# NTHU-LSALAB/KubeShare

Measured on AMD Instinct MI355X. Metric: aggregate images/sec, co-located shared-GPU pods, higher is better.
Workload: dtype bf16; 1 GPU; model=resnet50, global_batch=512, image_size=224, parallelism=2 pods @ request=0.5, 2/GPU, pods_per_gpu=2, miopen_find=False, lease_accounting=sampled-busy

## Files before the change

kubeshare_amd/models/resnet.py:

```python
from __future__ import annotations

import torch
import torch.nn as nn

from .conv import LowpConv2d
from .pool import FusedMaxPool2d


class Bottleneck(nn.Module):
    expansion = 4
    fused_ops = False

    def __init__(self, in_ch: int, width: int, stride: int = 1):
        super().__init__()
        out_ch = width * self.expansion
        self.conv1 = LowpConv2d(in_ch, width, 1, bias=False)
        self.bn1 = nn.BatchNorm2d(width)
        self.conv2 = LowpConv2d(width, width, 3, stride=stride, padding=1,
                                bias=False)
        self.bn2 = nn.BatchNorm2d(width)
        self.conv3 = LowpConv2d(width, out_ch, 1, bias=False)
        self.bn3 = nn.BatchNorm2d(out_ch)
        self.relu = nn.ReLU(inplace=True)
        self.down = None
        if stride != 1 or in_ch != out_ch:
            self.down = nn.Sequential(
                LowpConv2d(in_ch, out_ch, 1, stride=stride, bias=False),
                nn.BatchNorm2d(out_ch),
            )

    def forward(self, x):
        pair = isinstance(x, tuple)
        x, x_id = x if pair else (x, x)
        if self.fused_ops:
            from .. import ops
            identity = x_id if self.down is None else \
                ops.bn_relu(self.down[0](x_id), self.down[1], relu=False)
            out = ops.bn_relu(self.conv1(x), self.bn1)
            out = ops.bn_relu(self.conv2(out), self.bn2)
            return ops.bn_relu(self.conv3(out), self.bn3, res=identity,
                               fork=pair)
        identity = x_id if self.down is None else self.down(x_id)
        out = self.relu(self.bn1(self.conv1(x)))
        out = self.relu(self.bn2(self.conv2(out)))
        out = self.bn3(self.conv3(out))
        out = self.relu(out + identity)
        return (out, out) if pair else out


class BasicBlock(nn.Module):
    expansion = 1
    fused_ops = False

    def __init__(self, in_ch: int, width: int, stride: int = 1):
        super().__init__()
        self.conv1 = LowpConv2d(in_ch, width, 3, stride=stride, padding=1,
                                bias=False)
        self.bn1 = nn.BatchNorm2d(width)
        self.conv2 = LowpConv2d(width, width, 3, padding=1, bias=False)
        self.bn2 = nn.BatchNorm2d(width)
        self.relu = nn.ReLU(inplace=True)
        self.down = None
        if stride != 1 or in_ch != width:
            self.down = nn.Sequential(
                LowpConv2d(in_ch, width, 1, stride=stride, bias=False),
                nn.BatchNorm2d(width),
            )

    def forward(self, x):
        pair = isinstance(x, tuple)
        x, x_id = x if pair else (x, x)
        if self.fused_ops:
            from .. import ops
            identity = x_id if self.down is None else \
                ops.bn_relu(self.down[0](x_id), self.down[1], relu=False)
            out = ops.bn_relu(self.conv1(x), self.bn1)
            return ops.bn_relu(self.conv2(out), self.bn2, res=identity,
                               fork=pair)
        identity = x_id if self.down is None else self.down(x_id)
        out = self.relu(self.bn1(self.conv1(x)))
        out = self.bn2(self.conv2(out))
        out = self.relu(out + identity)
        return (out, out) if pair else out


class ResNet(nn.Module):
    fused_ops = False

    def __init__(self, block, layers, num_classes: int = 1000):
        super().__init__()
        self.in_ch = 64
        self.conv1 = LowpConv2d(3, 64, 7, stride=2, padding=3, bias=False)
        self.bn1 = nn.BatchNorm2d(64)
        self.relu = nn.ReLU(inplace=True)
        self.maxpool = FusedMaxPool2d(3, stride=2, padding=1)
        self.layer1 = self._make_layer(block, 64, layers[0])
        self.layer2 = self._make_layer(block, 128, layers[1], stride=2)
        self.layer3 = self._make_layer(block, 256, layers[2], stride=2)
        self.layer4 = self._make_layer(block, 512, layers[3], stride=2)
        self.avgpool = nn.AdaptiveAvgPool2d(1)
        self.fc = nn.Linear(512 * block.expansion, num_classes)
        for m in self.modules():
            if isinstance(m, nn.Conv2d):
                nn.init.kaiming_normal_(m.weight, mode="fan_out",
                                        nonlinearity="relu")
            elif isinstance(m, nn.BatchNorm2d):
                nn.init.ones_(m.weight)
                nn.init.zeros_(m.bias)
        self._lowp_convs = [m for m in self.modules()
                            if isinstance(m, LowpConv2d)]

    def _make_layer(self, block, width, n, stride=1):
        layers = [block(self.in_ch, width, stride)]
        self.in_ch = width * block.expansion
        layers += [block(self.in_ch, width) for _ in range(n - 1)]
        return nn.Sequential(*layers)

    def forward(self, x):
        if not self.fused_ops:
            return self._forward(x)
        from .. import ops
        staged = ops.stage_lowp_weights(self._lowp_convs)
        try:
            return self._forward(x)
        finally:
            ops.clear_lowp_weights(staged)

    def _forward(self, x):
        if self.fused_ops:
            from .. import ops
            x = self.maxpool(ops.PendingBNReLU(self.conv1(x), self.bn1))
            if ops.bn_fork_enabled():
                x = (x, x)
        else:
            x = self.maxpool(self.relu(self.bn1(self.conv1(x))))
        x = self.layer4(self.layer3(self.layer2(self.layer1(x))))
        if isinstance(x, tuple):
            x = x[0]
        x = torch.flatten(self.avgpool(x), 1)
        return self.fc(x)


def resnet18(num_classes: int = 1000) -> ResNet:
    return ResNet(BasicBlock, [2, 2, 2, 2], num_classes)


def resnet50(num_classes: int = 1000) -> ResNet:
    return ResNet(Bottleneck, [3, 4, 6, 3], num_classes)
```

kubeshare_amd/ops/__init__.py:

```python
from __future__ import annotations

import os

_HERE = os.path.dirname(os.path.abspath(__file__))
_BUILD_DIR = os.path.join(_HERE, "_build")
_SRCS = [os.path.join(_HERE, "hip", "ks_ops.hip"),
         os.path.join(_HERE, "hip", "bn_relu.hip"),
         os.path.join(_HERE, "hip", "pool.hip"),
         os.path.join(_HERE, "hip", "bn_pool.hip"),
         os.path.join(_HERE, "hip", "bias_relu.hip"),
         os.path.join(_HERE, "hip", "cast.hip")]

_ext = None


def build_extension(verbose: bool = False):
    import torch
    from torch.utils import cpp_extension

    os.environ.setdefault("PYTORCH_ROCM_ARCH", "gfx950")
    os.makedirs(_BUILD_DIR, exist_ok=True)
    return cpp_extension.load(
        name="ks_ops",
        sources=_SRCS,
        build_directory=_BUILD_DIR,
        extra_cflags=["-O3"],
        verbose=verbose,
        is_python_module=True,
    )


def _load():
    global _ext
    if _ext is not None:
        return _ext
    import torch

    so = os.path.join(_BUILD_DIR, "ks_ops.so")
    if os.path.exists(so):
        import importlib.util

        spec = importlib.util.spec_from_file_location("ks_ops", so)
        mod = importlib.util.module_from_spec(spec)
        spec.loader.exec_module(mod)
        _ext = mod
        return _ext
    if torch.cuda.is_available():
        _ext = build_extension()
        return _ext
    raise ImportError(
        "kubeshare_amd.ops extension not built; run __graft_entry__.build()")


def burn(ms: float, blocks: int = 1024, threads: int = 256):
    _load().burn(float(ms), blocks, threads)


class FusedSGD:

    def __init__(self, params, lr: float, momentum: float = 0.9,
                 weight_decay: float = 0.0, graph_mode: str = "auto"):
        import torch

        self.params = [p for p in params if p.requires_grad]
        self.lr = lr
        self.momentum = momentum
        self.weight_decay = weight_decay
        self.momenta = [torch.zeros_like(p) for p in self.params]
        self._graph_mode = graph_mode
        self._multi = os.environ.get("KUBESHARE_SGD_MULTI", "1") != "0"
        self._step_graph = None
        self._graph_ptrs = None

    def _graphable(self):
        import torch
        if self._graph_mode == "off" or not torch.cuda.is_available():
            return False
        if os.environ.get("KUBESHARE_SGD_GRAPH", "1") == "0":
            return False
        return all(p.grad is not None and p.grad.is_cuda
                   for p in self.params)

    def _ptrs(self):
        return tuple(
            (p.data_ptr(), v.data_ptr(),
             p.grad.data_ptr() if p.grad is not None else 0)
            for p, v in zip(self.params, self.momenta))

    def zero_grad(self, set_to_none: bool = True):
        for p in self.params:
            if set_to_none:
                p.grad = None
            elif p.grad is not None:
                p.grad.zero_()

    def _launch(self):
        ext = _load()
        if self._multi:
            ext.sgd_momentum_multi_(
                [p.data for p in self.params],
                [p.grad for p in self.params], self.momenta,
                self.lr, self.momentum, self.weight_decay)
            return
        ps, gs, vs = [], [], []
        for p, v in zip(self.params, self.momenta):
            if p.grad is None:
                continue
            ps.append(p.data)
            gs.append(p.grad)
            vs.append(v)
        ext.sgd_momentum_(ps, gs, vs, self.lr, self.momentum,
                          self.weight_decay)

    def _capture(self):
        import torch
        ptrs = self._ptrs()
        step_g = torch.cuda.CUDAGraph()
        with torch.cuda.graph(step_g):
            self._launch()
        self._step_graph = step_g
        self._graph_ptrs = ptrs

    def step(self):
        if self._step_graph is not None and \
                self._graph_ptrs == self._ptrs():
            self._step_graph.replay()
            return
        self._launch()
        if self._step_graph is None and self._graph_mode == "auto" and \
                self._graphable():
            try:
                self._capture()
            except Exception:
                self._graph_mode = "off"


def _bn_relu_autograd():
    global _BNReLUFn
    if _BNReLUFn is not None:
        return _BNReLUFn
    import torch

    class BNReLUFn(torch.autograd.Function):

        @staticmethod
        def forward(ctx, x, res, weight, bias, running_mean, running_var,
                    training, momentum, eps, relu, fork=False):
            ext = _load()
            w32 = weight.float()
            b32 = bias.float()
            ctx.set_materialize_grads(False)
            ctx.with_res = res is not None
            ctx.relu = relu
            ctx.wdtype = weight.dtype
            ctx.legacy_reduce = bn_reduce_legacy()
            if training:
                y, mean, invstd = ext.bn_relu_fwd_train(
                    x, w32, b32, running_mean, running_var, momentum, eps,
                    res, relu, ctx.legacy_reduce)
                ctx.save_for_backward(x, y, w32, b32, mean, invstd)
            else:
                y = ext.bn_relu_fwd_eval(x, w32, b32, running_mean.float(),
                                         running_var.float(), eps, res, relu)
                ctx.save_for_backward(x, y, w32, b32, running_mean.float(),
                                      (running_var.float() + eps).rsqrt())
            return (y, y.view_as(y)) if fork else y

        @staticmethod
        def backward(ctx, dy, dy2=None):
            ext = _load()
            x, y, w32, b32, mean, invstd = ctx.saved_tensors
            if dy is None:
                dy, dy2 = dy2, None
            if dy is None:
                return (None,) * 11
            out = ext.bn_relu_bwd(x, y, dy, w32, b32, mean, invstd,
                                  ctx.with_res, ctx.relu, dy2,
                                  ctx.legacy_reduce)
            dx, dscale, dbias = out[0], out[1], out[2]
            dres = out[3] if ctx.with_res else None
            return (dx, dres, dscale.to(ctx.wdtype), dbias.to(ctx.wdtype),
                    None, None, None, None, None, None, None)

    _BNReLUFn = BNReLUFn
    return BNReLUFn


_BNReLUFn = None


def bn_fork_enabled() -> bool:
    return os.environ.get("KUBESHARE_BN_FORK", "1") != "0"


def bn_reduce_legacy() -> bool:
    return os.environ.get("KUBESHARE_BN_REDUCE", "") == "legacy"


def bn_relu(x, bn, res=None, relu=True, fork=False):
    import torch

    supported = (x.dtype == torch.bfloat16 and x.size(1) % 8 == 0
                 and x.size(1) <= 2048 and x.is_cuda
                 and x.is_contiguous(memory_format=torch.channels_last))
    if supported and res is not None and res.dtype != torch.bfloat16:
        res = res.to(torch.bfloat16)
    if not supported:
        y = torch.nn.functional.batch_norm(
            x, bn.running_mean, bn.running_var, bn.weight, bn.bias,
            bn.training, bn.momentum, bn.eps)
        if res is not None:
            y = y + res
        y = torch.relu(y) if relu else y
        return (y, y) if fork else y
    if res is not None and not res.is_contiguous(
            memory_format=torch.channels_last):
        res = res.contiguous(memory_format=torch.channels_last)
    fn = _bn_relu_autograd()
    return fn.apply(x, res, bn.weight, bn.bias, bn.running_mean,
                    bn.running_var, bn.training, bn.momentum, bn.eps, relu,
                    fork)


_CastWeightsFn = None


def _cast_weights_autograd():
    global _CastWeightsFn
    if _CastWeightsFn is not None:
        return _CastWeightsFn
    import torch

    class CastWeightsFn(torch.autograd.Function):

        @staticmethod
        def forward(ctx, *weights):
            ctx.set_materialize_grads(False)
            return tuple(_load().cast_f32_to_bf16_multi(list(weights)))

        @staticmethod
        def backward(ctx, *grads):
            out = list(grads)
            idx = [i for i, g in enumerate(grads)
                   if g is not None and g.dtype == torch.bfloat16]
            if idx:
                cast = _load().cast_bf16_to_f32_multi(
                    [grads[i] for i in idx])
                for i, g in zip(idx, cast):
                    out[i] = g
            return tuple(out)

    _CastWeightsFn = CastWeightsFn
    return CastWeightsFn


def cast_weights_bf16(weights):
    fn = _CastWeightsFn or _cast_weights_autograd()
    return fn.apply(*weights)


def lowp_weights_enabled() -> bool:
    return os.environ.get("KUBESHARE_LOWP_WEIGHTS", "1") != "0"


def stage_lowp_weights(convs):
    import torch

    if not convs or not lowp_weights_enabled():
        return []
    if not torch.is_autocast_enabled("cuda") or \
            torch.get_autocast_dtype("cuda") != torch.bfloat16:
        return []
    weights = [m.weight for m in convs]
    if not all(w.is_cuda and w.dtype == torch.float32 for w in weights):
        return []
    for m, w in zip(convs, cast_weights_bf16(weights)):
        m._lowp_weight = w
    return convs


def clear_lowp_weights(convs):
    for m in convs:
        m._lowp_weight = None


_POOL_CONFIGS = ((3, 2, 1), (2, 2, 0))
_MaxPoolNHWCFn = None


def _pool_int(v):
    if type(v) is int:
        return v
    if isinstance(v, (tuple, list)) and len(v) == 2 and v[0] == v[1] \
            and type(v[0]) is int:
        return v[0]
    return None


def _pool_cfg(kernel_size, stride, padding):
    if stride is None or stride == () or stride == []:
        stride = kernel_size
    return (_pool_int(kernel_size), _pool_int(stride), _pool_int(padding))


def _pool_cfg_supported(x, cfg) -> bool:
    import torch

    if cfg not in _POOL_CONFIGS or x.dim() != 4:
        return False
    n, c, h, w = x.shape
    k, _, p = cfg
    return (x.is_cuda and x.dtype == torch.bfloat16
            and c % 8 == 0 and 8 <= c <= 2048 and n >= 1
            and h + 2 * p >= k and w + 2 * p >= k
            and n * h * w < 2 ** 31
            and x.is_contiguous(memory_format=torch.channels_last))


def fused_pool_enabled() -> bool:
    return os.environ.get("KUBESHARE_FUSED_POOL", "1") != "0"


def max_pool_supported(x, kernel_size, stride=None, padding=0) -> bool:
    return _pool_cfg_supported(x, _pool_cfg(kernel_size, stride, padding))


def _max_pool_autograd():
    global _MaxPoolNHWCFn
    if _MaxPoolNHWCFn is not None:
        return _MaxPoolNHWCFn
    import torch
    from torch.autograd.function import once_differentiable

    class MaxPoolNHWCFn(torch.autograd.Function):

        @staticmethod
        def forward(ctx, x, k, s, p, want_idx):
            out = _load().max_pool_nhwc_fwd(x, k, s, p, want_idx)
            if want_idx:
                ctx.save_for_backward(out[1])
                ctx.input_sizes = list(x.shape)
                ctx.cfg = (k, s, p)
            return out[0]

        @staticmethod
        @once_differentiable
        def backward(ctx, dy):
            (idx,) = ctx.saved_tensors
            if not dy.is_contiguous(memory_format=torch.channels_last):
                dy = dy.contiguous(memory_format=torch.channels_last)
            k, s, p = ctx.cfg
            dx = _load().max_pool_nhwc_bwd(dy, idx, ctx.input_sizes,
                                           k, s, p)
            return dx, None, None, None, None

    _MaxPoolNHWCFn = MaxPoolNHWCFn
    return MaxPoolNHWCFn


def max_pool_nhwc(x, kernel_size, stride=None, padding=0):
    import torch

    cfg = _pool_cfg(kernel_size, stride, padding)
    if not _pool_cfg_supported(x, cfg):
        return torch.nn.functional.max_pool2d(x, kernel_size, stride,
                                              padding)
    want_idx = torch.is_grad_enabled() and x.requires_grad
    fn = _MaxPoolNHWCFn or _max_pool_autograd()
    return fn.apply(x, *cfg, want_idx)


_BNReLUMaxPoolNHWCFn = None


def bn_pool_enabled() -> bool:
    return os.environ.get("KUBESHARE_BN_POOL", "1") != "0"


def bn_relu_pool_supported(x, kernel_size, stride=None, padding=0) -> bool:
    return _pool_cfg_supported(x, _pool_cfg(kernel_size, stride, padding))


def _bn_relu_pool_autograd():
    global _BNReLUMaxPoolNHWCFn
    if _BNReLUMaxPoolNHWCFn is not None:
        return _BNReLUMaxPoolNHWCFn
    import torch
    from torch.autograd.function import once_differentiable

    class BNReLUMaxPoolNHWCFn(torch.autograd.Function):

        @staticmethod
        def forward(ctx, x, weight, bias, running_mean, running_var,
                    training, momentum, eps, k, s, p, want_idx):
            ext = _load()
            w32 = weight.float()
            b32 = bias.float()
            if not training:
                return ext.bn_relu_pool_fwd_eval(
                    x, w32, b32, running_mean.float(), running_var.float(),
                    eps, k, s, p)[0]
            legacy = bn_reduce_legacy()
            out = ext.bn_relu_pool_fwd_train(
                x, w32, b32, running_mean, running_var, momentum, eps,
                k, s, p, want_idx, legacy)
            if want_idx:
                ctx.save_for_backward(x, out[3], out[1], out[2], w32, b32)
                ctx.cfg = (k, s, p)
                ctx.wdtype = weight.dtype
                ctx.legacy_reduce = legacy
            return out[0]

        @staticmethod
        @once_differentiable
        def backward(ctx, dy):
            x, idx, mean, invstd, w32, b32 = ctx.saved_tensors
            if not dy.is_contiguous(memory_format=torch.channels_last):
                dy = dy.contiguous(memory_format=torch.channels_last)
            dx, dscale, dbias = _load().bn_relu_pool_bwd(
                x, dy, idx, w32, b32, mean, invstd, *ctx.cfg,
                ctx.legacy_reduce)
            return (dx, dscale.to(ctx.wdtype), dbias.to(ctx.wdtype)) + \
                (None,) * 9

    _BNReLUMaxPoolNHWCFn = BNReLUMaxPoolNHWCFn
    return BNReLUMaxPoolNHWCFn


def bn_relu_pool(x, bn, kernel_size, stride=None, padding=0):
    import torch

    cfg = _pool_cfg(kernel_size, stride, padding)
    fused = bn_pool_enabled() and _pool_cfg_supported(x, cfg)
    want_idx = False
    if fused:
        want_idx = torch.is_grad_enabled() and (
            x.requires_grad or bn.weight.requires_grad
            or bn.bias.requires_grad)
        fused = bn.training or not want_idx
    if not fused:
        return max_pool_nhwc(bn_relu(x, bn), kernel_size, stride, padding)
    fn = _BNReLUMaxPoolNHWCFn or _bn_relu_pool_autograd()
    return fn.apply(x, bn.weight, bn.bias, bn.running_mean, bn.running_var,
                    bn.training, bn.momentum, bn.eps, *cfg, want_idx)


_BiasReLUFn = None
_BiasReLUMaxPoolNHWCFn = None


def bias_relu_enabled() -> bool:
    return os.environ.get("KUBESHARE_BIAS_RELU", "1") != "0"


def bias_relu_supported(x) -> bool:
    import torch

    if x.dim() != 4:
        return False
    n, c, h, w = x.shape
    return (x.is_cuda and x.dtype == torch.bfloat16
            and c % 8 == 0 and 8 <= c <= 2048
            and n >= 1 and h >= 1 and w >= 1 and n * h * w < 2 ** 31
            and x.is_contiguous(memory_format=torch.channels_last))


def bias_relu_pool_supported(x, kernel_size, stride=None, padding=0) -> bool:
    return _pool_cfg_supported(x, _pool_cfg(kernel_size, stride, padding))


def _bias_relu_autograd():
    global _BiasReLUFn
    if _BiasReLUFn is not None:
        return _BiasReLUFn
    import torch
    from torch.autograd.function import once_differentiable

    class BiasReLUFn(torch.autograd.Function):

        @staticmethod
        def forward(ctx, x, bias):
            y = _load().bias_relu_fwd(
                x, bias.detach().float().contiguous())
            ctx.save_for_backward(y)
            ctx.bdtype = bias.dtype
            return y

        @staticmethod
        @once_differentiable
        def backward(ctx, dy):
            (y,) = ctx.saved_tensors
            if not dy.is_contiguous(memory_format=torch.channels_last):
                dy = dy.contiguous(memory_format=torch.channels_last)
            dx, db = _load().bias_relu_bwd(dy, y)
            return dx, db.to(ctx.bdtype)

    _BiasReLUFn = BiasReLUFn
    return BiasReLUFn


def _bias_relu_pool_autograd():
    global _BiasReLUMaxPoolNHWCFn
    if _BiasReLUMaxPoolNHWCFn is not None:
        return _BiasReLUMaxPoolNHWCFn
    import torch
    from torch.autograd.function import once_differentiable

    class BiasReLUMaxPoolNHWCFn(torch.autograd.Function):

        @staticmethod
        def forward(ctx, x, bias, k, s, p, want_idx):
            out = _load().bias_relu_pool_fwd(
                x, bias.detach().float().contiguous(), k, s, p, want_idx)
            if want_idx:
                ctx.save_for_backward(out[1], out[0])
                ctx.input_sizes = list(x.shape)
                ctx.cfg = (k, s, p)
                ctx.bdtype = bias.dtype
            return out[0]

        @staticmethod
        @once_differentiable
        def backward(ctx, dy):
            idx, y = ctx.saved_tensors
            if not dy.is_contiguous(memory_format=torch.channels_last):
                dy = dy.contiguous(memory_format=torch.channels_last)
            dx, db = _load().bias_relu_pool_bwd(dy, idx, y, ctx.input_sizes,
                                                *ctx.cfg)
            return dx, db.to(ctx.bdtype), None, None, None, None

    _BiasReLUMaxPoolNHWCFn = BiasReLUMaxPoolNHWCFn
    return BiasReLUMaxPoolNHWCFn


def bias_relu(x, bias):
    import torch

    if not bias_relu_supported(x) or not bias.is_cuda:
        return torch.relu(x + bias.to(x.dtype).view(1, -1, 1, 1))
    fn = _BiasReLUFn or _bias_relu_autograd()
    return fn.apply(x, bias)


def bias_relu_pool(x, bias, kernel_size, stride=None, padding=0):
    import torch

    cfg = _pool_cfg(kernel_size, stride, padding)
    if not _pool_cfg_supported(x, cfg) or not bias.is_cuda:
        if bias_relu_supported(x) and bias.is_cuda:
            return max_pool_nhwc(bias_relu(x, bias), kernel_size, stride,
                                 padding)
        y = torch.relu(x + bias.to(x.dtype).view(1, -1, 1, 1))
        return torch.nn.functional.max_pool2d(y, kernel_size, stride,
                                              padding)
    want_idx = torch.is_grad_enabled() and (x.requires_grad
                                            or bias.requires_grad)
    fn = _BiasReLUMaxPoolNHWCFn or _bias_relu_pool_autograd()
    return fn.apply(x, bias, *cfg, want_idx)


class PendingBNReLU:

    __slots__ = ("x", "bn")

    def __init__(self, x, bn):
        self.x = x
        self.bn = bn

    def materialize(self):
        return bn_relu(self.x, self.bn)


def fuse_model(model):
    _load()
    for m in model.modules():
        if hasattr(m, "fused_ops"):
            m.fused_ops = True
    return model
```

kubeshare_amd/ops/hip/bn_common.h:

```cpp
#pragma once
#include <hip/hip_runtime.h>
#include <torch/extension.h>

typedef __attribute__((ext_vector_type(8))) unsigned short ushort8;
typedef __attribute__((ext_vector_type(8))) float float8;

#define KS_BN_BLOCK 512
#define KS_BN_UNROLL 4

__device__ __forceinline__ float bf16_to_f32(unsigned short u) {
  union {
    unsigned int i;
    float f;
  } v;
  v.i = ((unsigned int)u) << 16;
  return v.f;
}

__device__ __forceinline__ unsigned short f32_to_bf16(float f) {
  union {
    float f;
    unsigned int i;
  } v;
  v.f = f;
  unsigned int lsb = (v.i >> 16) & 1;
  v.i += 0x7fffu + lsb;
  return (unsigned short)(v.i >> 16);
}

__device__ __forceinline__ float bn_affine(float x, float s, float b) {
  return fmaf(x, s, b);
}

__device__ __forceinline__ unsigned short bn_relu_bf16(float f) {
  return f32_to_bf16(f < 0.f ? 0.f : f);
}

__device__ __forceinline__ float bn_mul_add_unfused(float acc, float a,
                                                    float b) {
#pragma clang fp contract(off)
  float prod = a * b;
  return acc + prod;
}

template <bool GROUPED>
__device__ __forceinline__ float bn_acc_dscale(float acc, float g, float xhat,
                                               int j) {
  return (GROUPED && j >= 6) ? bn_mul_add_unfused(acc, g, xhat)
                             : fmaf(g, xhat, acc);
}

struct BnGeom {
  long long M;
  int C, CG, blocks, stat_blocks;
};

BnGeom bn_geom_of(const torch::Tensor& x);

void bn_launch_fwd_stats(const torch::Tensor& x, const BnGeom& g,
                         const torch::Tensor& weight,
                         const torch::Tensor& bias, float* running_mean,
                         float* running_var, torch::Tensor& save_mean,
                         torch::Tensor& save_invstd, torch::Tensor& scale,
                         torch::Tensor& biasf, double momentum, double eps,
                         bool legacy_reduce, hipStream_t stream);

void bn_launch_bwd_reduce(const float* part, int nblocks, int C, float* out0,
                          float* out1, bool legacy_reduce,
                          hipStream_t stream);

void bn_launch_reduce_one(const float* part, int nblocks, int C, float* out,
                          hipStream_t stream);

void bn_launch_fold_eval(const torch::Tensor& weight,
                         const torch::Tensor& bias,
                         const torch::Tensor& rmean,
                         const torch::Tensor& rvar, torch::Tensor& scale,
                         torch::Tensor& biasf, int C, double eps,
                         hipStream_t stream);
```

kubeshare_amd/ops/hip/bn_pool.hip:

```cpp
#include <hip/hip_runtime.h>
#include <torch/extension.h>
#include <ATen/cuda/CUDAContext.h>

#include <vector>

#include "bn_common.h"

#define KS_BNP_FWD_BLOCK 256
#define KS_BNP_U_321 1
#define KS_BNP_U_220 2

template <int K, int S, bool WANT_IDX>
__global__ void __launch_bounds__(KS_BNP_FWD_BLOCK)
bn_pool_fwd_kernel(const ushort8* __restrict__ x, ushort8* __restrict__ y,
                   uint2* __restrict__ idx, const float* __restrict__ scale,
                   const float* __restrict__ biasf, int H, int W, int OH,
                   int OW, int pad, int M, int CG) {
  const int tid = threadIdx.x;
  const int cg = tid % CG;
  const int roff = tid / CG;
  const int rows_per_blk = KS_BNP_FWD_BLOCK / CG;
  if (roff >= rows_per_blk) return;
  const long long row64 = (long long)blockIdx.x * rows_per_blk + roff;
  if (row64 >= M) return;
  const int row = (int)row64;
  const int ow = row % OW;
  const int t = row / OW;
  const int oh = t % OH;
  const int n = t / OH;
  const int h0 = oh * S - pad;
  const int w0 = ow * S - pad;

  ushort8 v[K * K];
  bool ok[K * K];
#pragma unroll
  for (int kh = 0; kh < K; kh++) {
    const int h = h0 + kh;
    const int hc = h < 0 ? 0 : (h >= H ? H - 1 : h);
#pragma unroll
    for (int kw = 0; kw < K; kw++) {
      const int w = w0 + kw;
      const int wc = w < 0 ? 0 : (w >= W ? W - 1 : w);
      ok[kh * K + kw] = (h == hc) && (w == wc);
      const long long pix = ((long long)n * H + hc) * W + wc;
      v[kh * K + kw] = x[pix * CG + cg];
    }
  }
  float8 s, b;
#pragma unroll
  for (int j = 0; j < 8; j++) {
    s[j] = scale[cg * 8 + j];
    b[j] = biasf[cg * 8 + j];
  }

  const unsigned int q0 =
      (unsigned int)((h0 < 0 ? -h0 : 0) * K + (w0 < 0 ? -w0 : 0));
  float best[8];
  unsigned int code[8];
  ushort8 o;
#pragma unroll
  for (int j = 0; j < 8; j++) {
    best[j] = -INFINITY;
    code[j] = q0;
    o[j] = 0xff80u;
  }
#pragma unroll
  for (int q = 0; q < K * K; q++) {
    if (ok[q]) {
#pragma unroll
      for (int j = 0; j < 8; j++) {
        const unsigned short yb =
            bn_relu_bf16(bn_affine(bf16_to_f32(v[q][j]), s[j], b[j]));
        const float f = bf16_to_f32(yb);
        if (f > best[j] || f != f) {
          best[j] = f;
          o[j] = yb;
          code[j] = q;
        }
      }
    }
  }

  const long long k = (long long)row * CG + cg;
  y[k] = o;
  if (WANT_IDX) {
    uint2 c;
    c.x = code[0] | (code[1] << 8) | (code[2] << 16) | (code[3] << 24);
    c.y = code[4] | (code[5] << 8) | (code[6] << 16) | (code[7] << 24);
    idx[k] = c;
  }
}

template <int K, int S>
struct PoolGather {
  static constexpr int NW = (K + S - 1) / S;
  ushort8 g[NW * NW];
  uint2 c[NW * NW];
  unsigned int want[NW * NW];
  bool ok[NW * NW];

  __device__ __forceinline__ void load(const ushort8* __restrict__ dy,
                                       const uint2* __restrict__ idx,
                                       int row, int H, int W, int OH, int OW,
                                       int pad, int CG, int cg) {
    const int w = row % W;
    const int t = row / W;
    const int h = t % H;
    const int n = t / H;
    const int th = h + pad - K + 1;
    const int tw = w + pad - K + 1;
    const int oh_lo = th <= 0 ? 0 : (th + S - 1) / S;
    const int ow_lo = tw <= 0 ? 0 : (tw + S - 1) / S;
    int oh_hi = (h + pad) / S;
    int ow_hi = (w + pad) / S;
    oh_hi = oh_hi < OH ? oh_hi : OH - 1;
    ow_hi = ow_hi < OW ? ow_hi : OW - 1;
#pragma unroll
    for (int a = 0; a < NW; a++) {
      const int oh = oh_lo + a;
      const int ohc = oh < OH ? oh : OH - 1;
#pragma unroll
      for (int b = 0; b < NW; b++) {
        const int ow = ow_lo + b;
        const int owc = ow < OW ? ow : OW - 1;
        const int q = a * NW + b;
        ok[q] = oh <= oh_hi && ow <= ow_hi;
        want[q] =
            (unsigned int)((h + pad - oh * S) * K + (w + pad - ow * S));
        const long long k =
            (((long long)n * OH + ohc) * OW + owc) * CG + cg;
        g[q] = dy[k];
        c[q] = idx[k];
      }
    }
  }

  __device__ __forceinline__ float grad(int j) const {
    float acc = 0.f;
#pragma unroll
    for (int q = 0; q < NW * NW; q++) {
      if (ok[q]) {
        const unsigned int word = j < 4 ? c[q].x : c[q].y;
        const unsigned int code = (word >> (8 * (j & 3))) & 0xffu;
        if (code == want[q]) acc += bf16_to_f32(g[q][j]);
      }
    }
    return bf16_to_f32(f32_to_bf16(acc));
  }
};

__device__ __forceinline__ bool bn_pool_relu_on(float xf, float sc,
                                                float bf) {
  const float f = fmaf(xf, sc, bf);
  return f32_to_bf16(f > 0.f ? f : 0.f) != 0;
}

__device__ __forceinline__ float bn_pool_xhat(float xf, float mu, float is) {
#pragma clang fp contract(off)
  return (xf - mu) * is;
}

__device__ __forceinline__ float bn_pool_dx(float w, float g, float db,
                                            float xhat, float ds) {
#pragma clang fp contract(off)
  const float t = g - db;
  return w * fmaf(-xhat, ds, t);
}

__device__ __forceinline__ float bn_pool_fold_scale(float w, float is) {
  return w * is;
}

__device__ __forceinline__ float bn_pool_fold_bias(float b, float mu,
                                                   float sc) {
  return fmaf(-mu, sc, b);
}

template <int K, int S, int U>
__global__ void __launch_bounds__(KS_BN_BLOCK)
bn_pool_bwd_stats_kernel(const ushort8* __restrict__ x,
                         const ushort8* __restrict__ dy,
                         const uint2* __restrict__ idx,
                         const float* __restrict__ mean,
                         const float* __restrict__ invstd,
                         const float* __restrict__ weight,
                         const float* __restrict__ bias,
                         float* __restrict__ part, int H, int W, int OH,
                         int OW, int pad, long long M, int CG) {
  static_assert(KS_BN_UNROLL % U == 0, "sub-batches must tile a group");
  __shared__ float s_red[KS_BN_BLOCK * 8];
  const int tid = threadIdx.x;
  const int cg = tid % CG;
  const int roff = tid / CG;
  const int rows_per_blk = KS_BN_BLOCK / CG;
  const bool active = roff < rows_per_blk;
  const long long stride = (long long)gridDim.x * rows_per_blk;
  float8 mu, is, sc, bf;
#pragma unroll
  for (int j = 0; j < 8; j++) {
    const int c = cg * 8 + j;
    mu[j] = mean[c];
    is[j] = invstd[c];
    sc[j] = bn_pool_fold_scale(weight[c], is[j]);
    bf[j] = bn_pool_fold_bias(bias[c], mu[j], sc[j]);
  }
  float8 adb = {0, 0, 0, 0, 0, 0, 0, 0};
  float8 ads = {0, 0, 0, 0, 0, 0, 0, 0};
  long long row = active ? (long long)blockIdx.x * rows_per_blk + roff : M;
  for (; row + (KS_BN_UNROLL - 1) * stride < M;
       row += KS_BN_UNROLL * stride) {
#pragma unroll 1
    for (int h = 0; h < KS_BN_UNROLL; h += U) {
      ushort8 xv[U];
      PoolGather<K, S> pg[U];
#pragma unroll
      for (int u = 0; u < U; u++) {
        const long long r = row + (h + u) * stride;
        xv[u] = x[r * CG + cg];
        pg[u].load(dy, idx, (int)r, H, W, OH, OW, pad, CG, cg);
      }
#pragma unroll
      for (int u = 0; u < U; u++)
#pragma unroll
        for (int j = 0; j < 8; j++) {
          const float xf = bf16_to_f32(xv[u][j]);
          float g = pg[u].grad(j);
          if (!bn_pool_relu_on(xf, sc[j], bf[j])) g = 0.f;
          adb[j] += g;
          ads[j] = bn_acc_dscale<true>(ads[j], g,
                                       bn_pool_xhat(xf, mu[j], is[j]), j);
        }
    }
  }
  for (; row < M; row += stride) {
    const ushort8 xv = x[row * CG + cg];
    PoolGather<K, S> pg;
    pg.load(dy, idx, (int)row, H, W, OH, OW, pad, CG, cg);
#pragma unroll
    for (int j = 0; j < 8; j++) {
      const float xf = bf16_to_f32(xv[j]);
      float g = pg.grad(j);
      if (!bn_pool_relu_on(xf, sc[j], bf[j])) g = 0.f;
      adb[j] += g;
      ads[j] = bn_acc_dscale<false>(ads[j], g,
                                    bn_pool_xhat(xf, mu[j], is[j]), j);
    }
  }

  const int C = CG * 8;
  float* db_part = part + (long long)blockIdx.x * C;
  float* ds_part = part + (long long)(gridDim.x + blockIdx.x) * C;
#pragma unroll
  for (int j = 0; j < 8; j++) s_red[tid * 8 + j] = adb[j];
  __syncthreads();
  if (tid < CG) {
    float8 t = {0, 0, 0, 0, 0, 0, 0, 0};
    for (int r = 0; r < rows_per_blk; r++)
#pragma unroll
      for (int j = 0; j < 8; j++) t[j] += s_red[(r * CG + tid) * 8 + j];
#pragma unroll
    for (int j = 0; j < 8; j++) db_part[tid * 8 + j] = t[j];
  }
  __syncthreads();
#pragma unroll
  for (int j = 0; j < 8; j++) s_red[tid * 8 + j] = ads[j];
  __syncthreads();
  if (tid < CG) {
    float8 t = {0, 0, 0, 0, 0, 0, 0, 0};
    for (int r = 0; r < rows_per_blk; r++)
#pragma unroll
      for (int j = 0; j < 8; j++) t[j] += s_red[(r * CG + tid) * 8 + j];
#pragma unroll
    for (int j = 0; j < 8; j++) ds_part[tid * 8 + j] = t[j];
  }
}

template <int K, int S, int U>
__global__ void __launch_bounds__(KS_BN_BLOCK)
bn_pool_bwd_apply_kernel(const ushort8* __restrict__ x,
                         const ushort8* __restrict__ dy,
                         const uint2* __restrict__ idx,
                         ushort8* __restrict__ dx,
                         const float* __restrict__ mean,
                         const float* __restrict__ invstd,
                         const float* __restrict__ weight,
                         const float* __restrict__ bias,
                         const float* __restrict__ dbias,
                         const float* __restrict__ dscale, int H, int W,
                         int OH, int OW, int pad, long long M, int CG) {
  static_assert(KS_BN_UNROLL % U == 0, "sub-batches must tile a group");
  const int tid = threadIdx.x;
  const int cg = tid % CG;
  const int roff = tid / CG;
  const int rows_per_blk = KS_BN_BLOCK / CG;
  const bool active = roff < rows_per_blk;
  const long long stride = (long long)gridDim.x * rows_per_blk;
  const float invM = 1.f / (float)M;
  float8 mu, is, sc, bf, db, ds;
#pragma unroll
  for (int j = 0; j < 8; j++) {
    const int c = cg * 8 + j;
    mu[j] = mean[c];
    is[j] = invstd[c];
    sc[j] = bn_pool_fold_scale(weight[c], is[j]);
    bf[j] = bn_pool_fold_bias(bias[c], mu[j], sc[j]);
    db[j] = dbias[c] * invM;
    ds[j] = dscale[c] * invM;
  }
  long long row = active ? (long long)blockIdx.x * rows_per_blk + roff : M;
  for (; row + (KS_BN_UNROLL - 1) * stride < M;
       row += KS_BN_UNROLL * stride) {
#pragma unroll 1
    for (int h = 0; h < KS_BN_UNROLL; h += U) {
      ushort8 xv[U];
      long long k[U];
      PoolGather<K, S> pg[U];
#pragma unroll
      for (int u = 0; u < U; u++) {
        const long long r = row + (h + u) * stride;
        k[u] = r * CG + cg;
        xv[u] = x[k[u]];
        pg[u].load(dy, idx, (int)r, H, W, OH, OW, pad, CG, cg);
      }
#pragma unroll
      for (int u = 0; u < U; u++) {
        ushort8 o;
#pragma unroll
        for (int j = 0; j < 8; j++) {
          const float xf = bf16_to_f32(xv[u][j]);
          float g = pg[u].grad(j);
          if (!bn_pool_relu_on(xf, sc[j], bf[j])) g = 0.f;
          o[j] = f32_to_bf16(bn_pool_dx(
              sc[j], g, db[j], bn_pool_xhat(xf, mu[j], is[j]), ds[j]));
        }
        dx[k[u]] = o;
      }
    }
  }
  for (; row < M; row += stride) {
    const long long k = row * CG + cg;
    const ushort8 xv = x[k];
    PoolGather<K, S> pg;
    pg.load(dy, idx, (int)row, H, W, OH, OW, pad, CG, cg);
    ushort8 o;
#pragma unroll
    for (int j = 0; j < 8; j++) {
      const float xf = bf16_to_f32(xv[j]);
      float g = pg.grad(j);
      if (!bn_pool_relu_on(xf, sc[j], bf[j])) g = 0.f;
      o[j] = f32_to_bf16(
          bn_pool_dx(sc[j], g, db[j], bn_pool_xhat(xf, mu[j], is[j]), ds[j]));
    }
    dx[k] = o;
  }
}

namespace {

struct BnPoolGeom {
  BnGeom bn;
  int N, H, W, OH, OW, pad;
  long long MO;
};

BnPoolGeom bn_pool_geom(const torch::Tensor& x, int64_t k, int64_t s,
                        int64_t p) {
  TORCH_CHECK((k == 3 && s == 2 && p == 1) || (k == 2 && s == 2 && p == 0),
              "bn_relu_pool: (k, s, p) must be (3, 2, 1) or (2, 2, 0)");
  TORCH_CHECK(x.is_cuda(), "bn_relu_pool: GPU tensor expected");
  BnPoolGeom g;
  g.bn = bn_geom_of(x);
  const int64_t N = x.size(0), H = x.size(2), W = x.size(3);
  TORCH_CHECK(g.bn.C >= 8 && g.bn.C <= KS_BNP_FWD_BLOCK * 8,
              "bn_relu_pool: C must be a multiple of 8 in [8, 2048]");
  TORCH_CHECK(N >= 1 && H + 2 * p >= k && W + 2 * p >= k,
              "bn_relu_pool: empty output");
  TORCH_CHECK(N * H * W < (1LL << 31),
              "bn_relu_pool: N*H*W must fit 32 bits");
  g.N = (int)N;
  g.H = (int)H;
  g.W = (int)W;
  g.OH = (int)((H + 2 * p - k) / s + 1);
  g.OW = (int)((W + 2 * p - k) / s + 1);
  g.pad = (int)p;
  g.MO = (long long)g.N * g.OH * g.OW;
  return g;
}

void check_params(const BnPoolGeom& g, const torch::Tensor& t,
                  const char* what) {
  TORCH_CHECK(t.is_cuda() && t.scalar_type() == at::kFloat &&
                  t.is_contiguous() && t.numel() == g.bn.C,
              "bn_relu_pool: ", what, " must be a contiguous f32 GPU tensor "
              "of C elements");
}

torch::Tensor launch_fwd(const torch::Tensor& x, const BnPoolGeom& g,
                         int64_t k, const torch::Tensor& scale,
                         const torch::Tensor& biasf, torch::Tensor idx,
                         hipStream_t stream) {
  auto y = at::empty({g.N, g.bn.C, g.OH, g.OW},
                     x.options().memory_format(at::MemoryFormat::ChannelsLast));
  const bool want_idx = idx.defined();
  const int rows_per_blk = KS_BNP_FWD_BLOCK / g.bn.CG;
  const unsigned int blocks =
      (unsigned int)((g.MO + rows_per_blk - 1) / rows_per_blk);
  auto launch = [&](auto kern) {
    hipLaunchKernelGGL(kern, dim3(blocks), dim3(KS_BNP_FWD_BLOCK), 0, stream,
                       reinterpret_cast<const ushort8*>(x.data_ptr()),
                       reinterpret_cast<ushort8*>(y.data_ptr()),
                       want_idx ? reinterpret_cast<uint2*>(idx.data_ptr())
                                : nullptr,
                       scale.data_ptr<float>(), biasf.data_ptr<float>(), g.H,
                       g.W, g.OH, g.OW, g.pad, (int)g.MO, g.bn.CG);
  };
  if (k == 3)
    want_idx ? launch(bn_pool_fwd_kernel<3, 2, true>)
             : launch(bn_pool_fwd_kernel<3, 2, false>);
  else
    want_idx ? launch(bn_pool_fwd_kernel<2, 2, true>)
             : launch(bn_pool_fwd_kernel<2, 2, false>);
  return y;
}

}

std::vector<torch::Tensor> bn_relu_pool_fwd_train(
    torch::Tensor x, torch::Tensor weight, torch::Tensor bias,
    torch::Tensor running_mean, torch::Tensor running_var, double momentum,
    double eps, int64_t k, int64_t s, int64_t p, bool want_idx,
    bool legacy_reduce) {
  BnPoolGeom g = bn_pool_geom(x, k, s, p);
  check_params(g, weight, "weight");
  check_params(g, bias, "bias");
  auto stream = at::cuda::getCurrentCUDAStream();
  auto f32 = x.options().dtype(at::kFloat);
  auto save_mean = at::empty({g.bn.C}, f32);
  auto save_invstd = at::empty({g.bn.C}, f32);
  auto scale = at::empty({g.bn.C}, f32);
  auto biasf = at::empty({g.bn.C}, f32);
  float* rmean_p =
      running_mean.defined() ? running_mean.data_ptr<float>() : nullptr;
  float* rvar_p =
      running_var.defined() ? running_var.data_ptr<float>() : nullptr;
  bn_launch_fwd_stats(x, g.bn, weight, bias, rmean_p, rvar_p, save_mean,
                      save_invstd, scale, biasf, momentum, eps, legacy_reduce,
                      stream.stream());
  torch::Tensor idx;
  if (want_idx)
    idx = at::empty({g.N, g.OH, g.OW, g.bn.C}, x.options().dtype(at::kByte));
  auto y = launch_fwd(x, g, k, scale, biasf, idx, stream.stream());
  if (!want_idx) return {y, save_mean, save_invstd};
  return {y, save_mean, save_invstd, idx};
}

std::vector<torch::Tensor> bn_relu_pool_fwd_eval(
    torch::Tensor x, torch::Tensor weight, torch::Tensor bias,
    torch::Tensor rmean, torch::Tensor rvar, double eps, int64_t k,
    int64_t s, int64_t p) {
  BnPoolGeom g = bn_pool_geom(x, k, s, p);
  check_params(g, weight, "weight");
  check_params(g, bias, "bias");
  check_params(g, rmean, "running_mean");
  check_params(g, rvar, "running_var");
  auto stream = at::cuda::getCurrentCUDAStream();
  auto f32 = x.options().dtype(at::kFloat);
  auto scale = at::empty({g.bn.C}, f32);
  auto biasf = at::empty({g.bn.C}, f32);
  bn_launch_fold_eval(weight, bias, rmean, rvar, scale, biasf, g.bn.C, eps,
                      stream.stream());
  return {launch_fwd(x, g, k, scale, biasf, torch::Tensor(),
                     stream.stream())};
}

std::vector<torch::Tensor> bn_relu_pool_bwd(
    torch::Tensor x, torch::Tensor dy, torch::Tensor idx,
    torch::Tensor weight, torch::Tensor bias, torch::Tensor mean,
    torch::Tensor invstd, int64_t k, int64_t s, int64_t p,
    bool legacy_reduce) {
  BnPoolGeom g = bn_pool_geom(x, k, s, p);
  check_params(g, weight, "weight");
  check_params(g, bias, "bias");
  check_params(g, mean, "mean");
  check_params(g, invstd, "invstd");
  TORCH_CHECK(dy.is_cuda() && dy.dim() == 4 &&
                  dy.scalar_type() == at::kBFloat16 && dy.size(0) == g.N &&
                  dy.size(1) == g.bn.C && dy.size(2) == g.OH &&
                  dy.size(3) == g.OW,
              "bn_relu_pool_bwd: dy must be bf16 (N, C, OH, OW)");
  TORCH_CHECK(idx.is_cuda() && idx.scalar_type() == at::kByte &&
                  idx.is_contiguous() && idx.dim() == 4 &&
                  idx.size(0) == g.N && idx.size(1) == g.OH &&
                  idx.size(2) == g.OW && idx.size(3) == g.bn.C,
              "bn_relu_pool_bwd: idx must be uint8 (N, OH, OW, C)");
  if (!dy.is_contiguous(at::MemoryFormat::ChannelsLast))
    dy = dy.contiguous(at::MemoryFormat::ChannelsLast);
  auto stream = at::cuda::getCurrentCUDAStream();
  auto f32 = x.options().dtype(at::kFloat);
  const BnGeom& b = g.bn;
  auto part = at::empty({(long long)2 * b.stat_blocks * b.C}, f32);
  auto red = at::empty({b.C * 2}, f32);
  float* dbias_p = red.data_ptr<float>();
  float* dscale_p = dbias_p + b.C;
  auto dx = at::empty_like(x);

  auto launch_stats = [&](auto kern) {
    hipLaunchKernelGGL(kern, dim3(b.stat_blocks), dim3(KS_BN_BLOCK), 0,
                       stream.stream(),
                       reinterpret_cast<const ushort8*>(x.data_ptr()),
                       reinterpret_cast<const ushort8*>(dy.data_ptr()),
                       reinterpret_cast<const uint2*>(idx.data_ptr()),
                       mean.data_ptr<float>(), invstd.data_ptr<float>(),
                       weight.data_ptr<float>(), bias.data_ptr<float>(),
                       part.data_ptr<float>(), g.H, g.W, g.OH, g.OW, g.pad,
                       b.M, b.CG);
  };
  if (k == 3)
    launch_stats(bn_pool_bwd_stats_kernel<3, 2, KS_BNP_U_321>);
  else
    launch_stats(bn_pool_bwd_stats_kernel<2, 2, KS_BNP_U_220>);
  bn_launch_bwd_reduce(part.data_ptr<float>(), b.stat_blocks, b.C, dbias_p,
                       dscale_p, legacy_reduce, stream.stream());
  auto launch_apply = [&](auto kern) {
    hipLaunchKernelGGL(kern, dim3(b.blocks), dim3(KS_BN_BLOCK), 0,
                       stream.stream(),
                       reinterpret_cast<const ushort8*>(x.data_ptr()),
                       reinterpret_cast<const ushort8*>(dy.data_ptr()),
                       reinterpret_cast<const uint2*>(idx.data_ptr()),
                       reinterpret_cast<ushort8*>(dx.data_ptr()),
                       mean.data_ptr<float>(), invstd.data_ptr<float>(),
                       weight.data_ptr<float>(), bias.data_ptr<float>(),
                       dbias_p, dscale_p, g.H, g.W, g.OH, g.OW, g.pad, b.M,
                       b.CG);
  };
  if (k == 3)
    launch_apply(bn_pool_bwd_apply_kernel<3, 2, KS_BNP_U_321>);
  else
    launch_apply(bn_pool_bwd_apply_kernel<2, 2, KS_BNP_U_220>);
  return {dx, red.narrow(0, b.C, b.C), red.narrow(0, 0, b.C)};
}
```

kubeshare_amd/ops/hip/bn_relu.hip:

```cpp
#include <hip/hip_runtime.h>
#include <torch/extension.h>
#include <ATen/cuda/CUDAContext.h>

#include <vector>

#include "bn_common.h"

#define KS_BN_UNROLL_STATS 8
#define KS_BN_UNROLL_DY2 2

__global__ void bn_stats_kernel(const ushort8* __restrict__ x,
                                float* __restrict__ part,
                                long long M, int CG) {
  __shared__ float s_red[KS_BN_BLOCK * 8];
  const int tid = threadIdx.x;
  const int cg = tid % CG;
  const int roff = tid / CG;
  const int rows_per_blk = KS_BN_BLOCK / CG;
  const bool active = roff < rows_per_blk;
  const long long stride = (long long)gridDim.x * rows_per_blk;

  float8 acc = {0, 0, 0, 0, 0, 0, 0, 0};
  float8 acc2 = {0, 0, 0, 0, 0, 0, 0, 0};
  long long row = active ? (long long)blockIdx.x * rows_per_blk + roff : M;
  for (; row + (KS_BN_UNROLL_STATS - 1) * stride < M;
       row += KS_BN_UNROLL_STATS * stride) {
    ushort8 v[KS_BN_UNROLL_STATS];
#pragma unroll
    for (int u = 0; u < KS_BN_UNROLL_STATS; u++)
      v[u] = x[(row + u * stride) * CG + cg];
#pragma unroll
    for (int u = 0; u < KS_BN_UNROLL_STATS; u++)
#pragma unroll
      for (int j = 0; j < 8; j++) {
        float f = bf16_to_f32(v[u][j]);
        acc[j] += f;
        acc2[j] += f * f;
      }
  }
  for (; row < M; row += stride) {
    ushort8 v = x[row * CG + cg];
#pragma unroll
    for (int j = 0; j < 8; j++) {
      float f = bf16_to_f32(v[j]);
      acc[j] += f;
      acc2[j] += f * f;
    }
  }

  const int C = CG * 8;
  float* sum_part = part + (long long)blockIdx.x * C;
  float* sq_part = part + (long long)(gridDim.x + blockIdx.x) * C;
#pragma unroll
  for (int j = 0; j < 8; j++) s_red[tid * 8 + j] = acc[j];
  __syncthreads();
  if (tid < CG) {
    float8 t = {0, 0, 0, 0, 0, 0, 0, 0};
    for (int r = 0; r < rows_per_blk; r++)
#pragma unroll
      for (int j = 0; j < 8; j++) t[j] += s_red[(r * CG + tid) * 8 + j];
#pragma unroll
    for (int j = 0; j < 8; j++) sum_part[tid * 8 + j] = t[j];
  }
  __syncthreads();
#pragma unroll
  for (int j = 0; j < 8; j++) s_red[tid * 8 + j] = acc2[j];
  __syncthreads();
  if (tid < CG) {
    float8 t = {0, 0, 0, 0, 0, 0, 0, 0};
    for (int r = 0; r < rows_per_blk; r++)
#pragma unroll
      for (int j = 0; j < 8; j++) t[j] += s_red[(r * CG + tid) * 8 + j];
#pragma unroll
    for (int j = 0; j < 8; j++) sq_part[tid * 8 + j] = t[j];
  }
}

__global__ void bn_reduce_partials_kernel(const float* __restrict__ part,
                                          int nblocks, int C,
                                          float* __restrict__ out0,
                                          float* __restrict__ out1) {
  const int lane = threadIdx.x;
  const int c = blockIdx.x * blockDim.y + threadIdx.y;
  if (c >= C) return;
  float a0 = 0.f, a1 = 0.f;
  for (int b = lane; b < nblocks; b += 64) {
    a0 += part[(long long)b * C + c];
    a1 += part[(long long)(nblocks + b) * C + c];
  }
#pragma unroll
  for (int off = 32; off > 0; off >>= 1) {
    a0 += __shfl_down(a0, off, 64);
    a1 += __shfl_down(a1, off, 64);
  }
  if (lane == 0) {
    out0[c] = a0;
    out1[c] = a1;
  }
}

struct BnFinalizeArgs {
  const float* __restrict__ weight;
  const float* __restrict__ bias;
  float* __restrict__ running_mean;
  float* __restrict__ running_var;
  float* __restrict__ save_mean;
  float* __restrict__ save_invstd;
  float* __restrict__ scale_out;
  float* __restrict__ bias_out;
  long long M;
  float momentum, eps;
};

__device__ __forceinline__ void bn_finalize_channel(const BnFinalizeArgs& f,
                                                    int c, float sum,
                                                    float sumsq) {
#pragma clang fp contract(off)
  const long long M = f.M;
  float mean = sum / (float)M;
  float var = fmaf(-mean, mean, sumsq / (float)M);
  var = var < 0.f ? 0.f : var;
  float invstd = rsqrtf(var + f.eps);
  f.save_mean[c] = mean;
  f.save_invstd[c] = invstd;
  if (f.running_mean) {
    float unbiased = M > 1 ? var * (float)M / (float)(M - 1) : var;
    const float keep = 1.f - f.momentum;
    float rm = keep * f.running_mean[c];
    float rv = keep * f.running_var[c];
    float nm = f.momentum * mean;
    float nv = f.momentum * unbiased;
    f.running_mean[c] = rm + nm;
    f.running_var[c] = rv + nv;
  }
  float s = f.weight[c] * invstd;
  f.scale_out[c] = s;
  f.bias_out[c] = fmaf(-mean, s, f.bias[c]);
}

#define KS_BN_RTILE 16
#define KS_BN_RLOADS 8

template <int TILE, bool FINALIZE, bool TWO = true>
__global__ void __launch_bounds__(64 * TILE)
bn_reduce_tile_kernel(const float* __restrict__ part, int nblocks, int C,
                      float* __restrict__ out0, float* __restrict__ out1,
                      const BnFinalizeArgs fin) {
  constexpr int NW = TILE;
  constexpr int QC = 64 / NW;
  static_assert(TILE == 8 || TILE == 16, "64 % TILE, 64 * TILE <= 1024");
  static_assert(TWO || !FINALIZE, "the finalize math needs both sums");
  __shared__ float s_a[2][NW][TILE];
  const int tid = threadIdx.x;
  const int lane = tid & 63;
  const int w = tid >> 6;
  const int cc = lane % TILE;
  const int L = w + NW * (lane / TILE);
  const int c = blockIdx.x * TILE + cc;
  const bool valid = c < C;
  const float* p0 = part + c;
  const float* p1 = part + (long long)nblocks * C + c;
  float a0 = 0.f, a1 = 0.f;
  for (int b0 = L; b0 < nblocks; b0 += 64 * KS_BN_RLOADS) {
    float v0[KS_BN_RLOADS], v1[KS_BN_RLOADS];
#pragma unroll
    for (int u = 0; u < KS_BN_RLOADS; u++) {
      const int b = b0 + 64 * u;
      const bool ok = valid && b < nblocks;
      v0[u] = ok ? p0[(long long)b * C] : 0.f;
      if (TWO) v1[u] = ok ? p1[(long long)b * C] : 0.f;
    }
#pragma unroll
    for (int u = 0; u < KS_BN_RLOADS; u++)
      if (b0 + 64 * u < nblocks) {
        a0 += v0[u];
        if (TWO) a1 += v1[u];
      }
  }
#pragma unroll
  for (int off = 32; off >= NW; off >>= 1) {
    a0 += __shfl_down(a0, off / NW * TILE, 64);
    if (TWO) a1 += __shfl_down(a1, off / NW * TILE, 64);
  }
  if (lane < TILE) {
    s_a[0][w][cc] = a0;
    if (TWO) s_a[1][w][cc] = a1;
  }
  __syncthreads();
  if (tid >= 64 * (TILE / QC)) return;
  const int l2 = lane / QC;
  const int cc2 = w * QC + lane % QC;
  a0 = s_a[0][l2][cc2];
  if (TWO) a1 = s_a[1][l2][cc2];
#pragma unroll
  for (int off = NW / 2; off > 0; off >>= 1) {
    a0 += __shfl_down(a0, off * QC, 64);
    if (TWO) a1 += __shfl_down(a1, off * QC, 64);
  }
  const int c2 = blockIdx.x * TILE + cc2;
  if (l2 != 0 || c2 >= C) return;
  if (FINALIZE) {
    bn_finalize_channel(fin, c2, a0, a1);
  } else {
    out0[c2] = a0;
    if (TWO) out1[c2] = a1;
  }
}

__global__ void bn_finalize_kernel(const float* __restrict__ sum,
                                   const float* __restrict__ sumsq,
                                   const float* __restrict__ weight,
                                   const float* __restrict__ bias,
                                   float* __restrict__ running_mean,
                                   float* __restrict__ running_var,
                                   float* __restrict__ save_mean,
                                   float* __restrict__ save_invstd,
                                   float* __restrict__ scale_out,
                                   float* __restrict__ bias_out,
                                   long long M, int C, float momentum,
                                   float eps) {
  int c = blockIdx.x * blockDim.x + threadIdx.x;
  if (c >= C) return;
  const BnFinalizeArgs f = {weight, bias, running_mean, running_var,
                            save_mean, save_invstd, scale_out, bias_out,
                            M, momentum, eps};
  bn_finalize_channel(f, c, sum[c], sumsq[c]);
}

template <bool WITH_RES, bool RELU = true>
__global__ void bn_apply_relu_kernel(const ushort8* __restrict__ x,
                                     const ushort8* __restrict__ res,
                                     ushort8* __restrict__ y,
                                     const float* __restrict__ scale,
                                     const float* __restrict__ biasf,
                                     long long M, int CG) {
  const int tid = threadIdx.x;
  const int cg = tid % CG;
  const int roff = tid / CG;
  const int rows_per_blk = KS_BN_BLOCK / CG;
  const bool active = roff < rows_per_blk;
  const long long stride = (long long)gridDim.x * rows_per_blk;
  float8 s, b;
#pragma unroll
  for (int j = 0; j < 8; j++) {
    s[j] = scale[cg * 8 + j];
    b[j] = biasf[cg * 8 + j];
  }
  long long row = active ? (long long)blockIdx.x * rows_per_blk + roff : M;
  for (; row + (KS_BN_UNROLL - 1) * stride < M;
       row += KS_BN_UNROLL * stride) {
    ushort8 v[KS_BN_UNROLL], r[KS_BN_UNROLL], o[KS_BN_UNROLL];
    long long k[KS_BN_UNROLL];
#pragma unroll
    for (int u = 0; u < KS_BN_UNROLL; u++) {
      k[u] = (row + u * stride) * CG + cg;
      v[u] = x[k[u]];
      if (WITH_RES) r[u] = res[k[u]];
    }
#pragma unroll
    for (int u = 0; u < KS_BN_UNROLL; u++) {
#pragma unroll
      for (int j = 0; j < 8; j++) {
        float f = bn_affine(bf16_to_f32(v[u][j]), s[j], b[j]);
        if (WITH_RES) f += bf16_to_f32(r[u][j]);
        o[u][j] = RELU ? bn_relu_bf16(f) : f32_to_bf16(f);
      }
      y[k[u]] = o[u];
    }
  }
  for (; row < M; row += stride) {
    const long long k = row * CG + cg;
    ushort8 v = x[k];
    ushort8 r;
    if (WITH_RES) r = res[k];
    ushort8 o;
#pragma unroll
    for (int j = 0; j < 8; j++) {
      float f = bn_affine(bf16_to_f32(v[j]), s[j], b[j]);
      if (WITH_RES) f += bf16_to_f32(r[j]);
      o[j] = RELU ? bn_relu_bf16(f) : f32_to_bf16(f);
    }
    y[k] = o;
  }
}

__device__ __forceinline__ float bn_join_grad(unsigned short a,
                                              unsigned short b) {
  return bf16_to_f32(f32_to_bf16(bf16_to_f32(a) + bf16_to_f32(b)));
}

template <bool WRITE_DYM, bool WITH_DY2 = false>
__global__ void bn_bwd_stats_kernel(const ushort8* __restrict__ x,
                                    const ushort8* __restrict__ y,
                                    const ushort8* __restrict__ dy,
                                    const ushort8* __restrict__ dy2,
                                    ushort8* __restrict__ dym_out,
                                    const float* __restrict__ mean,
                                    const float* __restrict__ invstd,
                                    float* __restrict__ part,
                                    long long M, int CG) {
  __shared__ float s_red[KS_BN_BLOCK * 8];
  const int tid = threadIdx.x;
  const int cg = tid % CG;
  const int roff = tid / CG;
  const int rows_per_blk = KS_BN_BLOCK / CG;
  const bool active = roff < rows_per_blk;
  const long long stride = (long long)gridDim.x * rows_per_blk;
  float8 mu, is;
#pragma unroll
  for (int j = 0; j < 8; j++) {
    mu[j] = mean[cg * 8 + j];
    is[j] = invstd[cg * 8 + j];
  }
  float8 adb = {0, 0, 0, 0, 0, 0, 0, 0};
  float8 ads = {0, 0, 0, 0, 0, 0, 0, 0};
  constexpr int U = WITH_DY2 ? KS_BN_UNROLL_DY2 : KS_BN_UNROLL;
  static_assert(KS_BN_UNROLL % U == 0, "sub-batches must tile a group");
  long long row = active ? (long long)blockIdx.x * rows_per_blk + roff : M;
  for (; row + (KS_BN_UNROLL - 1) * stride < M;
       row += KS_BN_UNROLL * stride) {
#pragma unroll 1
    for (int h = 0; h < KS_BN_UNROLL; h += U) {
      ushort8 xv[U], yv[U], gv[U];
      ushort8 g2[U];
      long long k[U];
#pragma unroll
      for (int u = 0; u < U; u++) {
        k[u] = (row + (h + u) * stride) * CG + cg;
        xv[u] = x[k[u]];
        yv[u] = y[k[u]];
        gv[u] = dy[k[u]];
        if (WITH_DY2) g2[u] = dy2[k[u]];
      }
#pragma unroll
      for (int u = 0; u < U; u++) {
        ushort8 dm;
#pragma unroll
        for (int j = 0; j < 8; j++) {
          float gin = WITH_DY2 ? bn_join_grad(gv[u][j], g2[u][j])
                               : bf16_to_f32(gv[u][j]);
          float g = bf16_to_f32(yv[u][j]) > 0.f ? gin : 0.f;
          float xhat = (bf16_to_f32(xv[u][j]) - mu[j]) * is[j];
          adb[j] += g;
          ads[j] = bn_acc_dscale<true>(ads[j], g, xhat, j);
          if (WRITE_DYM) dm[j] = f32_to_bf16(g);
        }
        if (WRITE_DYM) dym_out[k[u]] = dm;
      }
    }
  }
  for (; row < M; row += stride) {
    const long long k = row * CG + cg;
    ushort8 xv = x[k], yv = y[k], gv = dy[k];
    ushort8 g2;
    if (WITH_DY2) g2 = dy2[k];
    ushort8 dm;
#pragma unroll
    for (int j = 0; j < 8; j++) {
      float gin = WITH_DY2 ? bn_join_grad(gv[j], g2[j]) : bf16_to_f32(gv[j]);
      float g = bf16_to_f32(yv[j]) > 0.f ? gin : 0.f;
      float xhat = (bf16_to_f32(xv[j]) - mu[j]) * is[j];
      adb[j] += g;
      ads[j] = bn_acc_dscale<false>(ads[j], g, xhat, j);
      if (WRITE_DYM) dm[j] = f32_to_bf16(g);
    }
    if (WRITE_DYM) dym_out[k] = dm;
  }

  const int C = CG * 8;
  float* db_part = part + (long long)blockIdx.x * C;
  float* ds_part = part + (long long)(gridDim.x + blockIdx.x) * C;
#pragma unroll
  for (int j = 0; j < 8; j++) s_red[tid * 8 + j] = adb[j];
  __syncthreads();
  if (tid < CG) {
    float8 t = {0, 0, 0, 0, 0, 0, 0, 0};
    for (int r = 0; r < rows_per_blk; r++)
#pragma unroll
      for (int j = 0; j < 8; j++) t[j] += s_red[(r * CG + tid) * 8 + j];
#pragma unroll
    for (int j = 0; j < 8; j++) db_part[tid * 8 + j] = t[j];
  }
  __syncthreads();
#pragma unroll
  for (int j = 0; j < 8; j++) s_red[tid * 8 + j] = ads[j];
  __syncthreads();
  if (tid < CG) {
    float8 t = {0, 0, 0, 0, 0, 0, 0, 0};
    for (int r = 0; r < rows_per_blk; r++)
#pragma unroll
      for (int j = 0; j < 8; j++) t[j] += s_red[(r * CG + tid) * 8 + j];
#pragma unroll
    for (int j = 0; j < 8; j++) ds_part[tid * 8 + j] = t[j];
  }
}

template <bool RELU = true>
__global__ void bn_bwd_stats_noy_kernel(const ushort8* __restrict__ x,
                                        const ushort8* __restrict__ dy,
                                        const float* __restrict__ mean,
                                        const float* __restrict__ invstd,
                                        const float* __restrict__ weight,
                                        const float* __restrict__ bias,
                                        float* __restrict__ part,
                                        long long M, int CG) {
  __shared__ float s_red[KS_BN_BLOCK * 8];
  const int tid = threadIdx.x;
  const int cg = tid % CG;
  const int roff = tid / CG;
  const int rows_per_blk = KS_BN_BLOCK / CG;
  const bool active = roff < rows_per_blk;
  const long long stride = (long long)gridDim.x * rows_per_blk;
  float8 mu, is, sc, bf;
#pragma unroll
  for (int j = 0; j < 8; j++) {
    const int c = cg * 8 + j;
    mu[j] = mean[c];
    is[j] = invstd[c];
    sc[j] = weight[c] * is[j];
    bf[j] = bias[c] - mu[j] * sc[j];
  }
  float8 adb = {0, 0, 0, 0, 0, 0, 0, 0};
  float8 ads = {0, 0, 0, 0, 0, 0, 0, 0};
  long long row = active ? (long long)blockIdx.x * rows_per_blk + roff : M;
  for (; row + (KS_BN_UNROLL - 1) * stride < M;
       row += KS_BN_UNROLL * stride) {
    ushort8 xv[KS_BN_UNROLL], gv[KS_BN_UNROLL];
#pragma unroll
    for (int u = 0; u < KS_BN_UNROLL; u++) {
      const long long k = (row + u * stride) * CG + cg;
      xv[u] = x[k];
      gv[u] = dy[k];
    }
#pragma unroll
    for (int u = 0; u < KS_BN_UNROLL; u++)
#pragma unroll
      for (int j = 0; j < 8; j++) {
        float xf = bf16_to_f32(xv[u][j]);
        float g = bf16_to_f32(gv[u][j]);
        if (RELU) {
          float f = fmaf(xf, sc[j], bf[j]);
          if (!f32_to_bf16(f > 0.f ? f : 0.f)) g = 0.f;
        }
        adb[j] += g;
        ads[j] += g * ((xf - mu[j]) * is[j]);
      }
  }
  for (; row < M; row += stride) {
    const long long k = row * CG + cg;
    ushort8 xv = x[k], gv = dy[k];
#pragma unroll
    for (int j = 0; j < 8; j++) {
      float xf = bf16_to_f32(xv[j]);
      float g = bf16_to_f32(gv[j]);
      if (RELU) {
        float f = fmaf(xf, sc[j], bf[j]);
        if (!f32_to_bf16(f > 0.f ? f : 0.f)) g = 0.f;
      }
      adb[j] += g;
      ads[j] += g * ((xf - mu[j]) * is[j]);
    }
  }

  const int C = CG * 8;
  float* db_part = part + (long long)blockIdx.x * C;
  float* ds_part = part + (long long)(gridDim.x + blockIdx.x) * C;
#pragma unroll
  for (int j = 0; j < 8; j++) s_red[tid * 8 + j] = adb[j];
  __syncthreads();
  if (tid < CG) {
    float8 t = {0, 0, 0, 0, 0, 0, 0, 0};
    for (int r = 0; r < rows_per_blk; r++)
#pragma unroll
      for (int j = 0; j < 8; j++) t[j] += s_red[(r * CG + tid) * 8 + j];
#pragma unroll
    for (int j = 0; j < 8; j++) db_part[tid * 8 + j] = t[j];
  }
  __syncthreads();
#pragma unroll
  for (int j = 0; j < 8; j++) s_red[tid * 8 + j] = ads[j];
  __syncthreads();
  if (tid < CG) {
    float8 t = {0, 0, 0, 0, 0, 0, 0, 0};
    for (int r = 0; r < rows_per_blk; r++)
#pragma unroll
      for (int j = 0; j < 8; j++) t[j] += s_red[(r * CG + tid) * 8 + j];
#pragma unroll
    for (int j = 0; j < 8; j++) ds_part[tid * 8 + j] = t[j];
  }
}

template <bool RELU = true>
__global__ void bn_bwd_apply_noy_kernel(const ushort8* __restrict__ x,
                                        const ushort8* __restrict__ dy,
                                        ushort8* __restrict__ dx,
                                        const float* __restrict__ mean,
                                        const float* __restrict__ invstd,
                                        const float* __restrict__ weight,
                                        const float* __restrict__ bias,
                                        const float* __restrict__ dbias,
                                        const float* __restrict__ dscale,
                                        long long M, int CG) {
  const int tid = threadIdx.x;
  const int cg = tid % CG;
  const int roff = tid / CG;
  const int rows_per_blk = KS_BN_BLOCK / CG;
  const bool active = roff < rows_per_blk;
  const long long stride = (long long)gridDim.x * rows_per_blk;
  const float invM = 1.f / (float)M;
  float8 mu, is, sc, bf, w, db, ds;
#pragma unroll
  for (int j = 0; j < 8; j++) {
    const int c = cg * 8 + j;
    mu[j] = mean[c];
    is[j] = invstd[c];
    sc[j] = weight[c] * is[j];
    bf[j] = bias[c] - mu[j] * sc[j];
    w[j] = sc[j];
    db[j] = dbias[c] * invM;
    ds[j] = dscale[c] * invM;
  }
  long long row = active ? (long long)blockIdx.x * rows_per_blk + roff : M;
  for (; row + (KS_BN_UNROLL - 1) * stride < M;
       row += KS_BN_UNROLL * stride) {
    ushort8 xv[KS_BN_UNROLL], gv[KS_BN_UNROLL];
    long long k[KS_BN_UNROLL];
#pragma unroll
    for (int u = 0; u < KS_BN_UNROLL; u++) {
      k[u] = (row + u * stride) * CG + cg;
      xv[u] = x[k[u]];
      gv[u] = dy[k[u]];
    }
#pragma unroll
    for (int u = 0; u < KS_BN_UNROLL; u++) {
      ushort8 o;
#pragma unroll
      for (int j = 0; j < 8; j++) {
        float xf = bf16_to_f32(xv[u][j]);
        float g = bf16_to_f32(gv[u][j]);
        if (RELU) {
          float f = fmaf(xf, sc[j], bf[j]);
          if (!f32_to_bf16(f > 0.f ? f : 0.f)) g = 0.f;
        }
        float xhat = (xf - mu[j]) * is[j];
        o[j] = f32_to_bf16(w[j] * (g - db[j] - xhat * ds[j]));
      }
      dx[k[u]] = o;
    }
  }
  for (; row < M; row += stride) {
    const long long k = row * CG + cg;
    ushort8 xv = x[k], gv = dy[k];
    ushort8 o;
#pragma unroll
    for (int j = 0; j < 8; j++) {
      float xf = bf16_to_f32(xv[j]);
      float g = bf16_to_f32(gv[j]);
      if (RELU) {
        float f = fmaf(xf, sc[j], bf[j]);
        if (!f32_to_bf16(f > 0.f ? f : 0.f)) g = 0.f;
      }
      float xhat = (xf - mu[j]) * is[j];
      o[j] = f32_to_bf16(w[j] * (g - db[j] - xhat * ds[j]));
    }
    dx[k] = o;
  }
}

__global__ void bn_bwd_apply_dym_kernel(const ushort8* __restrict__ x,
                                        const ushort8* __restrict__ dym,
                                        ushort8* __restrict__ dx,
                                        const float* __restrict__ mean,
                                        const float* __restrict__ invstd,
                                        const float* __restrict__ weight,
                                        const float* __restrict__ dbias,
                                        const float* __restrict__ dscale,
                                        long long M, int CG) {
  const int tid = threadIdx.x;
  const int cg = tid % CG;
  const int roff = tid / CG;
  const int rows_per_blk = KS_BN_BLOCK / CG;
  const bool active = roff < rows_per_blk;
  const long long stride = (long long)gridDim.x * rows_per_blk;
  const float invM = 1.f / (float)M;
  float8 mu, is, w, db, ds;
#pragma unroll
  for (int j = 0; j < 8; j++) {
    const int c = cg * 8 + j;
    mu[j] = mean[c];
    is[j] = invstd[c];
    w[j] = weight[c] * is[j];
    db[j] = dbias[c] * invM;
    ds[j] = dscale[c] * invM;
  }
  long long row = active ? (long long)blockIdx.x * rows_per_blk + roff : M;
  for (; row + (KS_BN_UNROLL - 1) * stride < M;
       row += KS_BN_UNROLL * stride) {
    ushort8 xv[KS_BN_UNROLL], gv[KS_BN_UNROLL];
    long long k[KS_BN_UNROLL];
#pragma unroll
    for (int u = 0; u < KS_BN_UNROLL; u++) {
      k[u] = (row + u * stride) * CG + cg;
      xv[u] = x[k[u]];
      gv[u] = dym[k[u]];
    }
#pragma unroll
    for (int u = 0; u < KS_BN_UNROLL; u++) {
      ushort8 o;
#pragma unroll
      for (int j = 0; j < 8; j++) {
        float g = bf16_to_f32(gv[u][j]);
        float xhat = (bf16_to_f32(xv[u][j]) - mu[j]) * is[j];
        o[j] = f32_to_bf16(w[j] * (g - db[j] - xhat * ds[j]));
      }
      dx[k[u]] = o;
    }
  }
  for (; row < M; row += stride) {
    const long long k = row * CG + cg;
    ushort8 xv = x[k], gv = dym[k];
    ushort8 o;
#pragma unroll
    for (int j = 0; j < 8; j++) {
      float g = bf16_to_f32(gv[j]);
      float xhat = (bf16_to_f32(xv[j]) - mu[j]) * is[j];
      o[j] = f32_to_bf16(w[j] * (g - db[j] - xhat * ds[j]));
    }
    dx[k] = o;
  }
}

__global__ void bn_bwd_apply_kernel(const ushort8* __restrict__ x,
                                    const ushort8* __restrict__ y,
                                    const ushort8* __restrict__ dy,
                                    ushort8* __restrict__ dx,
                                    const float* __restrict__ mean,
                                    const float* __restrict__ invstd,
                                    const float* __restrict__ weight,
                                    const float* __restrict__ dbias,
                                    const float* __restrict__ dscale,
                                    long long M, int CG) {
  const int tid = threadIdx.x;
  const int cg = tid % CG;
  const int roff = tid / CG;
  const int rows_per_blk = KS_BN_BLOCK / CG;
  const bool active = roff < rows_per_blk;
  const long long stride = (long long)gridDim.x * rows_per_blk;
  const float invM = 1.f / (float)M;
  float8 mu, is, w, db, ds;
#pragma unroll
  for (int j = 0; j < 8; j++) {
    const int c = cg * 8 + j;
    mu[j] = mean[c];
    is[j] = invstd[c];
    w[j] = weight[c] * is[j];
    db[j] = dbias[c] * invM;
    ds[j] = dscale[c] * invM;
  }
  long long row = active ? (long long)blockIdx.x * rows_per_blk + roff : M;
  for (; row + (KS_BN_UNROLL - 1) * stride < M;
       row += KS_BN_UNROLL * stride) {
    ushort8 xv[KS_BN_UNROLL], yv[KS_BN_UNROLL], gv[KS_BN_UNROLL];
    long long k[KS_BN_UNROLL];
#pragma unroll
    for (int u = 0; u < KS_BN_UNROLL; u++) {
      k[u] = (row + u * stride) * CG + cg;
      xv[u] = x[k[u]];
      yv[u] = y[k[u]];
      gv[u] = dy[k[u]];
    }
#pragma unroll
    for (int u = 0; u < KS_BN_UNROLL; u++) {
      ushort8 o;
#pragma unroll
      for (int j = 0; j < 8; j++) {
        float g = bf16_to_f32(yv[u][j]) > 0.f ? bf16_to_f32(gv[u][j]) : 0.f;
        float xhat = (bf16_to_f32(xv[u][j]) - mu[j]) * is[j];
        o[j] = f32_to_bf16(w[j] * (g - db[j] - xhat * ds[j]));
      }
      dx[k[u]] = o;
    }
  }
  for (; row < M; row += stride) {
    const long long k = row * CG + cg;
    ushort8 xv = x[k], yv = y[k], gv = dy[k];
    ushort8 o;
#pragma unroll
    for (int j = 0; j < 8; j++) {
      float g = bf16_to_f32(yv[j]) > 0.f ? bf16_to_f32(gv[j]) : 0.f;
      float xhat = (bf16_to_f32(xv[j]) - mu[j]) * is[j];
      o[j] = f32_to_bf16(w[j] * (g - db[j] - xhat * ds[j]));
    }
    dx[k] = o;
  }
}

__global__ void bn_fold_eval_kernel(const float* __restrict__ weight,
                                    const float* __restrict__ bias,
                                    const float* __restrict__ rmean,
                                    const float* __restrict__ rvar,
                                    float* __restrict__ scale_out,
                                    float* __restrict__ bias_out, int C,
                                    float eps) {
  int c = blockIdx.x * blockDim.x + threadIdx.x;
  if (c >= C) return;
  float s = weight[c] * rsqrtf(rvar[c] + eps);
  scale_out[c] = s;
  bias_out[c] = bias[c] - rmean[c] * s;
}

BnGeom bn_geom_of(const torch::Tensor& x) {
  TORCH_CHECK(x.dim() == 4, "bn_relu: 4D NCHW tensor expected");
  TORCH_CHECK(x.scalar_type() == at::kBFloat16, "bn_relu: bf16 only");
  TORCH_CHECK(x.is_contiguous(at::MemoryFormat::ChannelsLast),
              "bn_relu: channels-last only");
  BnGeom g;
  g.C = (int)x.size(1);
  TORCH_CHECK(g.C % 8 == 0 && g.C <= KS_BN_BLOCK * 8,
              "bn_relu: C must be a multiple of 8 and <= 8*KS_BN_BLOCK");
  g.M = x.numel() / g.C;
  g.CG = g.C / 8;
  long long work = g.M * g.CG;
  long long blocks = (work + KS_BN_BLOCK - 1) / KS_BN_BLOCK;
  g.blocks = (int)std::min<long long>(blocks, 2048);
  g.stat_blocks = (int)std::min<long long>(blocks, 1024);
  if (g.stat_blocks < 1) g.stat_blocks = 1;
  return g;
}

void bn_launch_fwd_stats(const torch::Tensor& x, const BnGeom& g,
                         const torch::Tensor& weight,
                         const torch::Tensor& bias, float* rmean_p,
                         float* rvar_p, torch::Tensor& save_mean,
                         torch::Tensor& save_invstd, torch::Tensor& scale,
                         torch::Tensor& biasf, double momentum, double eps,
                         bool legacy_reduce, hipStream_t stream) {
  auto f32 = x.options().dtype(at::kFloat);
  auto part = at::empty({(long long)2 * g.stat_blocks * g.C}, f32);
  hipLaunchKernelGGL(bn_stats_kernel, dim3(g.stat_blocks),
                     dim3(KS_BN_BLOCK), 0, stream,
                     reinterpret_cast<const ushort8*>(x.data_ptr()),
                     part.data_ptr<float>(), g.M, g.CG);
  if (legacy_reduce) {
    auto sums = at::empty({2 * g.C}, f32);
    hipLaunchKernelGGL(bn_reduce_partials_kernel,
                       dim3((g.C + 3) / 4), dim3(64, 4), 0, stream,
                       part.data_ptr<float>(), g.stat_blocks, g.C,
                       sums.data_ptr<float>(), sums.data_ptr<float>() + g.C);
    int fb = (g.C + 255) / 256;
    hipLaunchKernelGGL(bn_finalize_kernel, dim3(fb), dim3(256), 0,
                       stream, sums.data_ptr<float>(),
                       sums.data_ptr<float>() + g.C,
                       weight.data_ptr<float>(), bias.data_ptr<float>(),
                       rmean_p, rvar_p, save_mean.data_ptr<float>(),
                       save_invstd.data_ptr<float>(),
                       scale.data_ptr<float>(), biasf.data_ptr<float>(), g.M,
                       g.C, (float)momentum, (float)eps);
  } else {
    const BnFinalizeArgs fin = {
        weight.data_ptr<float>(), bias.data_ptr<float>(), rmean_p, rvar_p,
        save_mean.data_ptr<float>(), save_invstd.data_ptr<float>(),
        scale.data_ptr<float>(), biasf.data_ptr<float>(), g.M,
        (float)momentum, (float)eps};
    hipLaunchKernelGGL((bn_reduce_tile_kernel<KS_BN_RTILE, true>),
                       dim3((g.C + KS_BN_RTILE - 1) / KS_BN_RTILE),
                       dim3(64 * KS_BN_RTILE), 0, stream,
                       part.data_ptr<float>(), g.stat_blocks, g.C,
                       (float*)nullptr, (float*)nullptr, fin);
  }
}

void bn_launch_bwd_reduce(const float* part, int nblocks, int C, float* out0,
                          float* out1, bool legacy_reduce,
                          hipStream_t stream) {
  if (legacy_reduce) {
    hipLaunchKernelGGL(bn_reduce_partials_kernel, dim3((C + 3) / 4),
                       dim3(64, 4), 0, stream, part, nblocks, C, out0, out1);
  } else {
    hipLaunchKernelGGL((bn_reduce_tile_kernel<KS_BN_RTILE, false>),
                       dim3((C + KS_BN_RTILE - 1) / KS_BN_RTILE),
                       dim3(64 * KS_BN_RTILE), 0, stream, part, nblocks, C,
                       out0, out1, BnFinalizeArgs{});
  }
}

void bn_launch_reduce_one(const float* part, int nblocks, int C, float* out,
                          hipStream_t stream) {
  hipLaunchKernelGGL((bn_reduce_tile_kernel<KS_BN_RTILE, false, false>),
                     dim3((C + KS_BN_RTILE - 1) / KS_BN_RTILE),
                     dim3(64 * KS_BN_RTILE), 0, stream, part, nblocks, C, out,
                     (float*)nullptr, BnFinalizeArgs{});
}

void bn_launch_fold_eval(const torch::Tensor& weight,
                         const torch::Tensor& bias,
                         const torch::Tensor& rmean,
                         const torch::Tensor& rvar, torch::Tensor& scale,
                         torch::Tensor& biasf, int C, double eps,
                         hipStream_t stream) {
  int fb = (C + 255) / 256;
  hipLaunchKernelGGL(bn_fold_eval_kernel, dim3(fb), dim3(256), 0, stream,
                     weight.data_ptr<float>(), bias.data_ptr<float>(),
                     rmean.data_ptr<float>(), rvar.data_ptr<float>(),
                     scale.data_ptr<float>(), biasf.data_ptr<float>(), C,
                     (float)eps);
}

std::vector<torch::Tensor> bn_relu_fwd_train(
    torch::Tensor x, torch::Tensor weight, torch::Tensor bias,
    torch::Tensor running_mean, torch::Tensor running_var, double momentum,
    double eps, c10::optional<torch::Tensor> res, bool relu,
    bool legacy_reduce) {
  BnGeom g = bn_geom_of(x);
  auto stream = at::cuda::getCurrentCUDAStream();
  auto f32 = x.options().dtype(at::kFloat);
  auto y = at::empty_like(x);
  auto save_mean = at::empty({g.C}, f32);
  auto save_invstd = at::empty({g.C}, f32);
  auto scale = at::empty({g.C}, f32);
  auto biasf = at::empty({g.C}, f32);
  float* rmean_p =
      running_mean.defined() ? running_mean.data_ptr<float>() : nullptr;
  float* rvar_p =
      running_var.defined() ? running_var.data_ptr<float>() : nullptr;
  bn_launch_fwd_stats(x, g, weight, bias, rmean_p, rvar_p, save_mean,
                      save_invstd, scale, biasf, momentum, eps, legacy_reduce,
                      stream.stream());
  auto launch_apply = [&](auto kern) {
    hipLaunchKernelGGL(kern, dim3(g.blocks), dim3(KS_BN_BLOCK), 0,
                       stream.stream(),
                       reinterpret_cast<const ushort8*>(x.data_ptr()),
                       res.has_value()
                           ? reinterpret_cast<const ushort8*>(res->data_ptr())
                           : nullptr,
                       reinterpret_cast<ushort8*>(y.data_ptr()),
                       scale.data_ptr<float>(), biasf.data_ptr<float>(), g.M,
                       g.CG);
  };
  if (res.has_value())
    relu ? launch_apply(bn_apply_relu_kernel<true, true>)
         : launch_apply(bn_apply_relu_kernel<true, false>);
  else
    relu ? launch_apply(bn_apply_relu_kernel<false, true>)
         : launch_apply(bn_apply_relu_kernel<false, false>);
  return {y, save_mean, save_invstd};
}

torch::Tensor bn_relu_fwd_eval(torch::Tensor x, torch::Tensor weight,
                               torch::Tensor bias, torch::Tensor rmean,
                               torch::Tensor rvar, double eps,
                               c10::optional<torch::Tensor> res, bool relu) {
  BnGeom g = bn_geom_of(x);
  auto stream = at::cuda::getCurrentCUDAStream();
  auto f32 = x.options().dtype(at::kFloat);
  auto scale = at::empty({g.C}, f32);
  auto biasf = at::empty({g.C}, f32);
  auto y = at::empty_like(x);
  bn_launch_fold_eval(weight, bias, rmean, rvar, scale, biasf, g.C, eps,
                      stream.stream());
  auto launch_apply = [&](auto kern) {
    hipLaunchKernelGGL(kern, dim3(g.blocks), dim3(KS_BN_BLOCK), 0,
                       stream.stream(),
                       reinterpret_cast<const ushort8*>(x.data_ptr()),
                       res.has_value()
                           ? reinterpret_cast<const ushort8*>(res->data_ptr())
                           : nullptr,
                       reinterpret_cast<ushort8*>(y.data_ptr()),
                       scale.data_ptr<float>(), biasf.data_ptr<float>(), g.M,
                       g.CG);
  };
  if (res.has_value())
    relu ? launch_apply(bn_apply_relu_kernel<true, true>)
         : launch_apply(bn_apply_relu_kernel<true, false>);
  else
    relu ? launch_apply(bn_apply_relu_kernel<false, true>)
         : launch_apply(bn_apply_relu_kernel<false, false>);
  return y;
}

std::vector<torch::Tensor> bn_relu_bwd(torch::Tensor x, torch::Tensor y,
                                       torch::Tensor dy, torch::Tensor weight,
                                       torch::Tensor bias, torch::Tensor mean,
                                       torch::Tensor invstd, bool need_dres,
                                       bool relu,
                                       c10::optional<torch::Tensor> dy2,
                                       bool legacy_reduce) {
  TORCH_CHECK(relu || !need_dres,
              "bn_relu_bwd: residual path requires the ReLU variant");
  BnGeom g = bn_geom_of(x);
  TORCH_CHECK(dy.sizes() == x.sizes() && y.sizes() == x.sizes() &&
                  dy.scalar_type() == at::kBFloat16,
              "bn_relu_bwd: dy must be bf16 of x's shape");
  bool fold_dy2 = false;
  if (dy2.has_value() && dy2->defined()) {
    TORCH_CHECK(dy2->sizes() == x.sizes(),
                "bn_relu_bwd: dy2 must have x's shape");
    fold_dy2 = need_dres && dy2->is_cuda() &&
               dy2->scalar_type() == at::kBFloat16 &&
               dy2->is_contiguous(at::MemoryFormat::ChannelsLast) &&
               dy.is_contiguous(at::MemoryFormat::ChannelsLast);
    if (!fold_dy2) dy = (dy + *dy2).to(at::kBFloat16);
  }
  auto stream = at::cuda::getCurrentCUDAStream();
  auto f32 = x.options().dtype(at::kFloat);
  auto part = at::empty({(long long)2 * g.stat_blocks * g.C}, f32);
  auto red = at::empty({g.C * 2}, f32);
  float* dbias_p = red.data_ptr<float>();
  float* dscale_p = dbias_p + g.C;
  auto dx = at::empty_like(x);
  torch::Tensor dres;
  if (!dy.is_contiguous(at::MemoryFormat::ChannelsLast))
    dy = dy.contiguous(at::MemoryFormat::ChannelsLast);
  auto launch_reduce = [&]() {
    bn_launch_bwd_reduce(part.data_ptr<float>(), g.stat_blocks, g.C, dbias_p,
                         dscale_p, legacy_reduce, stream.stream());
  };

  if (need_dres) {
    dres = at::empty_like(x);
    auto launch_rstats = [&](auto kern) {
      hipLaunchKernelGGL(kern, dim3(g.stat_blocks), dim3(KS_BN_BLOCK), 0,
                         stream.stream(),
                         reinterpret_cast<const ushort8*>(x.data_ptr()),
                         reinterpret_cast<const ushort8*>(y.data_ptr()),
                         reinterpret_cast<const ushort8*>(dy.data_ptr()),
                         fold_dy2 ? reinterpret_cast<const ushort8*>(
                                        dy2->data_ptr())
                                  : nullptr,
                         reinterpret_cast<ushort8*>(dres.data_ptr()),
                         mean.data_ptr<float>(), invstd.data_ptr<float>(),
                         part.data_ptr<float>(), g.M, g.CG);
    };
    fold_dy2 ? launch_rstats(bn_bwd_stats_kernel<true, true>)
             : launch_rstats(bn_bwd_stats_kernel<true, false>);
    launch_reduce();
    hipLaunchKernelGGL(bn_bwd_apply_dym_kernel, dim3(g.blocks),
                       dim3(KS_BN_BLOCK), 0, stream.stream(),
                       reinterpret_cast<const ushort8*>(x.data_ptr()),
                       reinterpret_cast<const ushort8*>(dres.data_ptr()),
                       reinterpret_cast<ushort8*>(dx.data_ptr()),
                       mean.data_ptr<float>(), invstd.data_ptr<float>(),
                       weight.data_ptr<float>(), dbias_p, dscale_p,
                       g.M, g.CG);
    auto dbias = red.narrow(0, 0, g.C);
    auto dscale = red.narrow(0, g.C, g.C);
    return {dx, dscale, dbias, dres};
  }
  auto launch_stats = [&](auto kern) {
    hipLaunchKernelGGL(kern, dim3(g.stat_blocks), dim3(KS_BN_BLOCK), 0,
                       stream.stream(),
                       reinterpret_cast<const ushort8*>(x.data_ptr()),
                       reinterpret_cast<const ushort8*>(dy.data_ptr()),
                       mean.data_ptr<float>(), invstd.data_ptr<float>(),
                       weight.data_ptr<float>(), bias.data_ptr<float>(),
                       part.data_ptr<float>(), g.M, g.CG);
  };
  relu ? launch_stats(bn_bwd_stats_noy_kernel<true>)
       : launch_stats(bn_bwd_stats_noy_kernel<false>);
  launch_reduce();
  auto launch_bapply = [&](auto kern) {
    hipLaunchKernelGGL(kern, dim3(g.blocks), dim3(KS_BN_BLOCK), 0,
                       stream.stream(),
                       reinterpret_cast<const ushort8*>(x.data_ptr()),
                       reinterpret_cast<const ushort8*>(dy.data_ptr()),
                       reinterpret_cast<ushort8*>(dx.data_ptr()),
                       mean.data_ptr<float>(), invstd.data_ptr<float>(),
                       weight.data_ptr<float>(), bias.data_ptr<float>(),
                       dbias_p, dscale_p, g.M, g.CG);
  };
  relu ? launch_bapply(bn_bwd_apply_noy_kernel<true>)
       : launch_bapply(bn_bwd_apply_noy_kernel<false>);
  auto dbias = red.narrow(0, 0, g.C);
  auto dscale = red.narrow(0, g.C, g.C);
  return {dx, dscale, dbias};
}
```

kubeshare_amd/ops/hip/ks_ops.hip:

```cpp
#include <hip/hip_runtime.h>
#include <torch/extension.h>
#include <ATen/cuda/CUDAContext.h>

#include <vector>

#define WAVE 64

__global__ void burn_kernel(long long ticks, float* sink) {
  long long start = wall_clock64();
  float acc = threadIdx.x * 1e-9f;
  while (wall_clock64() - start < ticks) {
#pragma unroll
    for (int i = 0; i < 64; i++) acc = fmaf(acc, 1.0000001f, 1e-12f);
  }
  if (acc == 12345.678f) sink[0] = acc;
}

void burn(double ms, int64_t blocks, int64_t threads) {
  long long ticks = (long long)(ms * 100000.0);
  auto stream = at::cuda::getCurrentCUDAStream();
  static float* sink = nullptr;
  if (!sink) {
    if (hipMalloc(&sink, sizeof(float)) != hipSuccess)
      throw std::runtime_error("burn: hipMalloc failed");
  }
  hipLaunchKernelGGL(burn_kernel, dim3((uint32_t)blocks),
                     dim3((uint32_t)threads), 0, stream.stream(), ticks,
                     sink);
}

template <typename T>
struct Vec4;
template <>
struct Vec4<float> {
  using type = float4;
};

__device__ __forceinline__ void sgd_mom_update(float& p, float g, float& v,
                                               float lr, float mu, float wd) {
  v = fmaf(wd, p, fmaf(mu, v, g));
  p = fmaf(-lr, v, p);
}

__device__ __forceinline__ void sgd_mom_update4(float4& p, const float4& g,
                                                float4& v, float lr, float mu,
                                                float wd) {
  sgd_mom_update(p.x, g.x, v.x, lr, mu, wd);
  sgd_mom_update(p.y, g.y, v.y, lr, mu, wd);
  sgd_mom_update(p.z, g.z, v.z, lr, mu, wd);
  sgd_mom_update(p.w, g.w, v.w, lr, mu, wd);
}

__global__ void sgd_mom_f32_kernel(float* __restrict__ p,
                                   const float* __restrict__ g,
                                   float* __restrict__ v, float lr, float mu,
                                   float wd, long long n) {
  long long i = (long long)blockIdx.x * blockDim.x + threadIdx.x;
  long long stride = (long long)gridDim.x * blockDim.x;
  long long n4 = n / 4;
  const float4* g4 = reinterpret_cast<const float4*>(g);
  float4* p4 = reinterpret_cast<float4*>(p);
  float4* v4 = reinterpret_cast<float4*>(v);
  for (long long k = i; k < n4; k += stride) {
    float4 pv = p4[k], gv = g4[k], vv = v4[k];
    sgd_mom_update4(pv, gv, vv, lr, mu, wd);
    v4[k] = vv;
    p4[k] = pv;
  }
  for (long long k = n4 * 4 + i; k < n; k += stride) {
    float pv = p[k], vv = v[k];
    sgd_mom_update(pv, g[k], vv, lr, mu, wd);
    v[k] = vv;
    p[k] = pv;
  }
}

#define KS_SGD_THREADS 256
#define KS_SGD_VPT 4
#define KS_SGD_CHUNK (KS_SGD_THREADS * KS_SGD_VPT * 4)
#define KS_SGD_MAX_TENSORS 110

struct SgdMultiArgs {
  float* p[KS_SGD_MAX_TENSORS];
  const float* g[KS_SGD_MAX_TENSORS];
  float* v[KS_SGD_MAX_TENSORS];
  long long n[KS_SGD_MAX_TENSORS];
  int blk[KS_SGD_MAX_TENSORS + 1];
  int count;
  float lr, mu, wd;
};
static_assert(sizeof(SgdMultiArgs) <= 4096,
              "SgdMultiArgs must fit the 4 KiB kernel-argument segment");

__global__ void __launch_bounds__(KS_SGD_THREADS)
sgd_mom_multi_f32_kernel(const SgdMultiArgs a) {
  const int b = blockIdx.x;
  int lo = 0, hi = a.count - 1;
  while (lo < hi) {
    int mid = (lo + hi + 1) >> 1;
    if (a.blk[mid] <= b) lo = mid; else hi = mid - 1;
  }
  float* __restrict__ p = a.p[lo];
  const float* __restrict__ g = a.g[lo];
  float* __restrict__ v = a.v[lo];
  const long long n = a.n[lo];
  const float lr = a.lr, mu = a.mu, wd = a.wd;
  const long long base = (long long)(b - a.blk[lo]) * KS_SGD_CHUNK;
  long long rem = n - base;
  const int len = rem < KS_SGD_CHUNK ? (int)rem : KS_SGD_CHUNK;
  p += base;
  g += base;
  v += base;
  const int tid = threadIdx.x;
  const bool vec = (((uintptr_t)p | (uintptr_t)g | (uintptr_t)v) & 15) == 0;
  if (vec) {
    const int len4 = len >> 2;
    const float4* g4 = reinterpret_cast<const float4*>(g);
    float4* p4 = reinterpret_cast<float4*>(p);
    float4* v4 = reinterpret_cast<float4*>(v);
    if (len == KS_SGD_CHUNK) {
      float4 pv[KS_SGD_VPT], gv[KS_SGD_VPT], vv[KS_SGD_VPT];
#pragma unroll
      for (int u = 0; u < KS_SGD_VPT; u++) {
        const int k = tid + u * KS_SGD_THREADS;
        pv[u] = p4[k];
        gv[u] = g4[k];
        vv[u] = v4[k];
      }
#pragma unroll
      for (int u = 0; u < KS_SGD_VPT; u++) {
        const int k = tid + u * KS_SGD_THREADS;
        sgd_mom_update4(pv[u], gv[u], vv[u], lr, mu, wd);
        v4[k] = vv[u];
        p4[k] = pv[u];
      }
      return;
    }
    for (int k = tid; k < len4; k += KS_SGD_THREADS) {
      float4 pv = p4[k], gv = g4[k], vv = v4[k];
      sgd_mom_update4(pv, gv, vv, lr, mu, wd);
      v4[k] = vv;
      p4[k] = pv;
    }
    for (int k = len4 * 4 + tid; k < len; k += KS_SGD_THREADS) {
      float pv = p[k], vv = v[k];
      sgd_mom_update(pv, g[k], vv, lr, mu, wd);
      v[k] = vv;
      p[k] = pv;
    }
    return;
  }
  for (int k = tid; k < len; k += KS_SGD_THREADS) {
    float pv = p[k], vv = v[k];
    sgd_mom_update(pv, g[k], vv, lr, mu, wd);
    v[k] = vv;
    p[k] = pv;
  }
}

void sgd_momentum_(std::vector<torch::Tensor> params,
                   std::vector<torch::Tensor> grads,
                   std::vector<torch::Tensor> momenta, double lr, double mu,
                   double wd) {
  auto stream = at::cuda::getCurrentCUDAStream();
  for (size_t t = 0; t < params.size(); t++) {
    auto& p = params[t];
    auto& g = grads[t];
    auto& v = momenta[t];
    TORCH_CHECK(p.is_cuda() && p.scalar_type() == at::kFloat &&
                    p.is_non_overlapping_and_dense() &&
                    g.sizes() == p.sizes() && g.strides() == p.strides() &&
                    v.strides() == p.strides() &&
                    g.scalar_type() == at::kFloat &&
                    v.scalar_type() == at::kFloat,
                "sgd_momentum_: f32 dense tensors with matching strides "
                "(any memory format: the update is elementwise over the "
                "flat storage)");
    long long n = p.numel();
    int threads = 256;
    int blocks = (int)std::min<long long>(2048, (n / 4 + threads - 1) / threads + 1);
    hipLaunchKernelGGL(sgd_mom_f32_kernel, dim3(blocks), dim3(threads), 0,
                       stream.stream(), p.data_ptr<float>(),
                       g.data_ptr<float>(), v.data_ptr<float>(), (float)lr,
                       (float)mu, (float)wd, n);
  }
}

int64_t sgd_momentum_multi_(std::vector<torch::Tensor> params,
                            std::vector<c10::optional<torch::Tensor>> grads,
                            std::vector<torch::Tensor> momenta, double lr,
                            double mu, double wd) {
  TORCH_CHECK(params.size() == grads.size() &&
                  params.size() == momenta.size(),
              "sgd_momentum_multi_: params, grads and momenta differ in "
              "length");
  auto stream = at::cuda::getCurrentCUDAStream();
  const long long max_blocks = 1LL << 30;
  SgdMultiArgs a = {};
  a.lr = (float)lr;
  a.mu = (float)mu;
  a.wd = (float)wd;
  a.count = 0;
  a.blk[0] = 0;
  int64_t launches = 0;
  std::vector<torch::Tensor> keep;
  auto flush = [&]() {
    if (a.count == 0) return;
    hipLaunchKernelGGL(sgd_mom_multi_f32_kernel, dim3(a.blk[a.count]),
                       dim3(KS_SGD_THREADS), 0, stream.stream(), a);
    launches++;
    a.count = 0;
  };
  for (size_t t = 0; t < params.size(); t++) {
    if (!grads[t].has_value() || !grads[t]->defined()) continue;
    auto& p = params[t];
    auto& v = momenta[t];
    torch::Tensor g = *grads[t];
    TORCH_CHECK(g.sizes() == p.sizes() && g.is_cuda() &&
                    g.scalar_type() == at::kFloat,
                "sgd_momentum_multi_: f32 CUDA gradient of the "
                "parameter's shape expected");
    if (g.strides() != p.strides()) {
      g = at::empty_like(p).copy_(g);
      keep.push_back(g);
    }
    TORCH_CHECK(p.is_cuda() && p.scalar_type() == at::kFloat &&
                    p.is_non_overlapping_and_dense() &&
                    g.sizes() == p.sizes() && g.strides() == p.strides() &&
                    v.strides() == p.strides() &&
                    g.scalar_type() == at::kFloat &&
                    v.scalar_type() == at::kFloat,
                "sgd_momentum_: f32 dense tensors with matching strides "
                "(any memory format: the update is elementwise over the "
                "flat storage)");
    TORCH_CHECK(v.is_cuda() && v.sizes() == p.sizes() &&
                    p.get_device() == stream.device_index() &&
                    g.get_device() == p.get_device() &&
                    v.get_device() == p.get_device(),
                "sgd_momentum_multi_: parameter, gradient and momentum "
                "must live on the current device and share a shape");
    const long long n = p.numel();
    if (n == 0) continue;
    const long long nb = (n + KS_SGD_CHUNK - 1) / KS_SGD_CHUNK;
    TORCH_CHECK(nb <= max_blocks, "sgd_momentum_multi_: tensor too large");
    if (a.count == KS_SGD_MAX_TENSORS || a.blk[a.count] + nb > max_blocks)
      flush();
    a.p[a.count] = p.data_ptr<float>();
    a.g[a.count] = g.data_ptr<float>();
    a.v[a.count] = v.data_ptr<float>();
    a.n[a.count] = n;
    a.blk[a.count + 1] = a.blk[a.count] + (int)nb;
    a.count++;
  }
  flush();
  return launches;
}

std::vector<torch::Tensor> bn_relu_fwd_train(
    torch::Tensor x, torch::Tensor weight, torch::Tensor bias,
    torch::Tensor running_mean, torch::Tensor running_var, double momentum,
    double eps, c10::optional<torch::Tensor> res, bool relu,
    bool legacy_reduce);
torch::Tensor bn_relu_fwd_eval(torch::Tensor x, torch::Tensor weight,
                               torch::Tensor bias, torch::Tensor rmean,
                               torch::Tensor rvar, double eps,
                               c10::optional<torch::Tensor> res, bool relu);
std::vector<torch::Tensor> bn_relu_bwd(torch::Tensor x, torch::Tensor y,
                                       torch::Tensor dy, torch::Tensor weight,
                                       torch::Tensor bias, torch::Tensor mean,
                                       torch::Tensor invstd, bool need_dres,
                                       bool relu,
                                       c10::optional<torch::Tensor> dy2,
                                       bool legacy_reduce);

std::vector<c10::optional<torch::Tensor>> cast_f32_to_bf16_multi(
    std::vector<c10::optional<torch::Tensor>> src);
std::vector<c10::optional<torch::Tensor>> cast_bf16_to_f32_multi(
    std::vector<c10::optional<torch::Tensor>> src);

std::vector<torch::Tensor> max_pool_nhwc_fwd(torch::Tensor x, int64_t k,
                                             int64_t s, int64_t p,
                                             bool want_idx);
torch::Tensor max_pool_nhwc_bwd(torch::Tensor dy, torch::Tensor idx,
                                std::vector<int64_t> input_sizes, int64_t k,
                                int64_t s, int64_t p);

std::vector<torch::Tensor> bn_relu_pool_fwd_train(
    torch::Tensor x, torch::Tensor weight, torch::Tensor bias,
    torch::Tensor running_mean, torch::Tensor running_var, double momentum,
    double eps, int64_t k, int64_t s, int64_t p, bool want_idx,
    bool legacy_reduce);
std::vector<torch::Tensor> bn_relu_pool_fwd_eval(
    torch::Tensor x, torch::Tensor weight, torch::Tensor bias,
    torch::Tensor rmean, torch::Tensor rvar, double eps, int64_t k,
    int64_t s, int64_t p);
std::vector<torch::Tensor> bn_relu_pool_bwd(
    torch::Tensor x, torch::Tensor dy, torch::Tensor idx,
    torch::Tensor weight, torch::Tensor bias, torch::Tensor mean,
    torch::Tensor invstd, int64_t k, int64_t s, int64_t p,
    bool legacy_reduce);

torch::Tensor bias_relu_fwd(torch::Tensor x, torch::Tensor bias);
std::vector<torch::Tensor> bias_relu_bwd(torch::Tensor dy, torch::Tensor y);
std::vector<torch::Tensor> bias_relu_pool_fwd(torch::Tensor x,
                                              torch::Tensor bias, int64_t k,
                                              int64_t s, int64_t p,
                                              bool want_idx);
std::vector<torch::Tensor> bias_relu_pool_bwd(
    torch::Tensor dy, torch::Tensor idx, torch::Tensor y,
    std::vector<int64_t> input_sizes, int64_t k, int64_t s, int64_t p);

PYBIND11_MODULE(TORCH_EXTENSION_NAME, m) {
  m.def("burn", &burn, "occupy the GPU for ~ms milliseconds",
        py::arg("ms"), py::arg("blocks") = 1024, py::arg("threads") = 256);
  m.def("sgd_momentum_", &sgd_momentum_,
        "fused SGD+momentum update (in-place)");
  m.def("sgd_momentum_multi_", &sgd_momentum_multi_,
        "fused SGD+momentum update of all tensors in as few launches as "
        "the kernel-argument limit allows; a None gradient skips its "
        "tensor; returns the number of launches");
  m.def("bn_relu_fwd_train", &bn_relu_fwd_train, py::arg("x"),
        py::arg("weight"), py::arg("bias"), py::arg("running_mean"),
        py::arg("running_var"), py::arg("momentum"), py::arg("eps"),
        py::arg("res"), py::arg("relu"), py::arg("legacy_reduce") = false);
  m.def("bn_relu_fwd_eval", &bn_relu_fwd_eval);
  m.def("bn_relu_bwd", &bn_relu_bwd, py::arg("x"), py::arg("y"),
        py::arg("dy"), py::arg("weight"), py::arg("bias"), py::arg("mean"),
        py::arg("invstd"), py::arg("need_dres"), py::arg("relu"),
        py::arg("dy2") = py::none(), py::arg("legacy_reduce") = false);
  m.def("cast_f32_to_bf16_multi", &cast_f32_to_bf16_multi,
        "f32 -> bf16 (torch rounding) of every tensor of a list in as few "
        "launches as the kernel-argument limit allows; None stays None");
  m.def("cast_bf16_to_f32_multi", &cast_bf16_to_f32_multi,
        "bf16 -> f32 of every tensor of a list; None stays None");
  m.def("max_pool_nhwc_fwd", &max_pool_nhwc_fwd);
  m.def("max_pool_nhwc_bwd", &max_pool_nhwc_bwd);
  m.def("bn_relu_pool_fwd_train", &bn_relu_pool_fwd_train, py::arg("x"),
        py::arg("weight"), py::arg("bias"), py::arg("running_mean"),
        py::arg("running_var"), py::arg("momentum"), py::arg("eps"),
        py::arg("k"), py::arg("s"), py::arg("p"), py::arg("want_idx"),
        py::arg("legacy_reduce") = false,
        "{y, mean, invstd} and, with want_idx, the one-byte window codes");
  m.def("bn_relu_pool_fwd_eval", &bn_relu_pool_fwd_eval,
        "{y} from the running statistics; no codes");
  m.def("bn_relu_pool_bwd", &bn_relu_pool_bwd, py::arg("x"), py::arg("dy"),
        py::arg("idx"), py::arg("weight"), py::arg("bias"), py::arg("mean"),
        py::arg("invstd"), py::arg("k"), py::arg("s"), py::arg("p"),
        py::arg("legacy_reduce") = false, "{dx, dscale, dbias}");
  m.def("bias_relu_fwd", &bias_relu_fwd, py::arg("x"), py::arg("bias"),
        "y = bf16(relu(f32(x) + bias)), bias f32");
  m.def("bias_relu_bwd", &bias_relu_bwd, py::arg("dy"), py::arg("y"),
        "{dx, db}");
  m.def("bias_relu_pool_fwd", &bias_relu_pool_fwd, py::arg("x"),
        py::arg("bias"), py::arg("k"), py::arg("s"), py::arg("p"),
        py::arg("want_idx"),
        "{y} and, with want_idx, the one-byte window codes");
  m.def("bias_relu_pool_bwd", &bias_relu_pool_bwd, py::arg("dy"),
        py::arg("idx"), py::arg("y"), py::arg("input_sizes"), py::arg("k"),
        py::arg("s"), py::arg("p"), "{dx, db}");
}
```

Measured before the change: 9145 images/s.

## Fuse downsample BN with residual BN-add-ReLU and save bit ReLU masks

Adds a bn_join kernel family that computes relu(bn(x) + bn_d(x_d)) in one pass for blocks with a downsample branch, with a joint backward that produces gradients for both BNs. This removes the separate downsample BN launch and the materialized identity tensor. It also stores a one-bit-per-element ReLU mask instead of the full bf16 output for residual BNs, so backward reads less memory and the saved activation footprint shrinks. The cost is more kernel code and extra state, and the numerics must stay matched (bf16 rounding of the identity, shared dbias).

```diff
diff --git a/kubeshare_amd/models/resnet.py b/kubeshare_amd/models/resnet.py
--- a/kubeshare_amd/models/resnet.py
+++ b/kubeshare_amd/models/resnet.py
@@ -34,11 +34,14 @@
         x, x_id = x if pair else (x, x)
         if self.fused_ops:
             from .. import ops
-            identity = x_id if self.down is None else \
-                ops.bn_relu(self.down[0](x_id), self.down[1], relu=False)
+            if self.down is not None:
+                x_d = self.down[0](x_id)
             out = ops.bn_relu(self.conv1(x), self.bn1)
             out = ops.bn_relu(self.conv2(out), self.bn2)
-            return ops.bn_relu(self.conv3(out), self.bn3, res=identity,
+            if self.down is not None:
+                return ops.bn_join(self.conv3(out), self.bn3, x_d,
+                                   self.down[1], fork=pair)
+            return ops.bn_relu(self.conv3(out), self.bn3, res=x_id,
                                fork=pair)
         identity = x_id if self.down is None else self.down(x_id)
         out = self.relu(self.bn1(self.conv1(x)))
@@ -72,10 +75,13 @@
         x, x_id = x if pair else (x, x)
         if self.fused_ops:
             from .. import ops
-            identity = x_id if self.down is None else \
-                ops.bn_relu(self.down[0](x_id), self.down[1], relu=False)
+            if self.down is not None:
+                x_d = self.down[0](x_id)
             out = ops.bn_relu(self.conv1(x), self.bn1)
-            return ops.bn_relu(self.conv2(out), self.bn2, res=identity,
+            if self.down is not None:
+                return ops.bn_join(self.conv2(out), self.bn2, x_d,
+                                   self.down[1], fork=pair)
+            return ops.bn_relu(self.conv2(out), self.bn2, res=x_id,
                                fork=pair)
         identity = x_id if self.down is None else self.down(x_id)
         out = self.relu(self.bn1(self.conv1(x)))
diff --git a/kubeshare_amd/ops/__init__.py b/kubeshare_amd/ops/__init__.py
--- a/kubeshare_amd/ops/__init__.py
+++ b/kubeshare_amd/ops/__init__.py
@@ -8,6 +8,7 @@
          os.path.join(_HERE, "hip", "bn_relu.hip"),
          os.path.join(_HERE, "hip", "pool.hip"),
          os.path.join(_HERE, "hip", "bn_pool.hip"),
+         os.path.join(_HERE, "hip", "bn_join.hip"),
          os.path.join(_HERE, "hip", "bias_relu.hip"),
          os.path.join(_HERE, "hip", "cast.hip")]
 
@@ -154,11 +155,15 @@
             ctx.relu = relu
             ctx.wdtype = weight.dtype
             ctx.legacy_reduce = bn_reduce_legacy()
+            ctx.masked = bool(training and relu and res is not None
+                              and bn_mask_enabled())
             if training:
-                y, mean, invstd = ext.bn_relu_fwd_train(
+                out = ext.bn_relu_fwd_train(
                     x, w32, b32, running_mean, running_var, momentum, eps,
-                    res, relu, ctx.legacy_reduce)
-                ctx.save_for_backward(x, y, w32, b32, mean, invstd)
+                    res, relu, ctx.legacy_reduce, ctx.masked)
+                y, mean, invstd = out[0], out[1], out[2]
+                ctx.save_for_backward(x, out[3] if ctx.masked else y, w32,
+                                      b32, mean, invstd)
             else:
                 y = ext.bn_relu_fwd_eval(x, w32, b32, running_mean.float(),
                                          running_var.float(), eps, res, relu)
@@ -174,9 +179,10 @@
                 dy, dy2 = dy2, None
             if dy is None:
                 return (None,) * 11
-            out = ext.bn_relu_bwd(x, y, dy, w32, b32, mean, invstd,
-                                  ctx.with_res, ctx.relu, dy2,
-                                  ctx.legacy_reduce)
+            out = ext.bn_relu_bwd(x, None if ctx.masked else y, dy, w32,
+                                  b32, mean, invstd, ctx.with_res, ctx.relu,
+                                  dy2, ctx.legacy_reduce,
+                                  y if ctx.masked else None)
             dx, dscale, dbias = out[0], out[1], out[2]
             dres = out[3] if ctx.with_res else None
             return (dx, dres, dscale.to(ctx.wdtype), dbias.to(ctx.wdtype),
@@ -195,6 +201,10 @@
 
 def bn_reduce_legacy() -> bool:
     return os.environ.get("KUBESHARE_BN_REDUCE", "") == "legacy"
+
+
+def bn_mask_enabled() -> bool:
+    return os.environ.get("KUBESHARE_BN_MASK", "1") != "0"
 
 
 def bn_relu(x, bn, res=None, relu=True, fork=False):
@@ -222,6 +232,83 @@
                     fork)
 
 
+_BNJoinFn = None
+
+
+def bn_join_enabled() -> bool:
+    return os.environ.get("KUBESHARE_BN_JOIN", "1") != "0"
+
+
+def _bn_join_autograd():
+    global _BNJoinFn
+    if _BNJoinFn is not None:
+        return _BNJoinFn
+    import torch
+
+    class BNJoinFn(torch.autograd.Function):
+
+        @staticmethod
+        def forward(ctx, x, x_d, weight, bias, running_mean, running_var,
+                    momentum, eps, weight_d, bias_d, running_mean_d,
+                    running_var_d, momentum_d, eps_d, fork):
+            ext = _load()
+            w32, b32 = weight.float(), bias.float()
+            wd32, bd32 = weight_d.float(), bias_d.float()
+            ctx.set_materialize_grads(False)
+            ctx.wdtype = weight.dtype
+            ctx.wdtype_d = weight_d.dtype
+            ctx.legacy_reduce = bn_reduce_legacy()
+            ctx.masked = bn_mask_enabled()
+            out = ext.bn_join_fwd_train(
+                x, w32, b32, running_mean, running_var, momentum, eps,
+                x_d, wd32, bd32, running_mean_d, running_var_d, momentum_d,
+                eps_d, ctx.masked, ctx.legacy_reduce)
+            y = out[0]
+            ctx.save_for_backward(x, x_d, out[5] if ctx.masked else y, w32,
+                                  wd32, *out[1:5])
+            return (y, y.view_as(y)) if fork else y
+
+        @staticmethod
+        def backward(ctx, dy, dy2=None):
+            x, x_d, ym, w32, wd32, mean, invstd, mean_d, invstd_d = \
+                ctx.saved_tensors
+            if dy is None:
+                dy, dy2 = dy2, None
+            if dy is None:
+                return (None,) * 15
+            dx, dx_d, dscale, dbias, dscale_d = _load().bn_join_bwd(
+                x, x_d, ym, dy, dy2, w32, wd32, mean, invstd, mean_d,
+                invstd_d, ctx.masked, ctx.legacy_reduce)
+            return (dx, dx_d, dscale.to(ctx.wdtype), dbias.to(ctx.wdtype),
+                    None, None, None, None, dscale_d.to(ctx.wdtype_d),
+                    dbias.clone().to(ctx.wdtype_d), None, None, None, None,
+                    None)
+
+    _BNJoinFn = BNJoinFn
+    return BNJoinFn
+
+
+def bn_join_supported(x, x_d) -> bool:
+    import torch
+
+    return (x.dim() == 4 and x.shape == x_d.shape
+            and x.size(1) % 8 == 0 and x.size(1) <= 2048
+            and all(t.is_cuda and t.dtype == torch.bfloat16
+                    and t.is_contiguous(memory_format=torch.channels_last)
+                    for t in (x, x_d)))
+
+
+def bn_join(x, bn, x_d, bn_d, fork=False):
+    if not (bn_join_enabled() and bn.training and bn_d.training
+            and bn_join_supported(x, x_d)):
+        return bn_relu(x, bn, res=bn_relu(x_d, bn_d, relu=False), fork=fork)
+    fn = _BNJoinFn or _bn_join_autograd()
+    return fn.apply(x, x_d, bn.weight, bn.bias, bn.running_mean,
+                    bn.running_var, bn.momentum, bn.eps, bn_d.weight,
+                    bn_d.bias, bn_d.running_mean, bn_d.running_var,
+                    bn_d.momentum, bn_d.eps, fork)
+
+
 _CastWeightsFn = None
 
 
diff --git a/kubeshare_amd/ops/hip/bn_common.h b/kubeshare_amd/ops/hip/bn_common.h
--- a/kubeshare_amd/ops/hip/bn_common.h
+++ b/kubeshare_amd/ops/hip/bn_common.h
@@ -50,12 +50,40 @@
                              : fmaf(g, xhat, acc);
 }
 
+__device__ __forceinline__ float bn_join_grad(unsigned short a,
+                                              unsigned short b) {
+  return bf16_to_f32(f32_to_bf16(bf16_to_f32(a) + bf16_to_f32(b)));
+}
+
+__device__ __forceinline__ float bn_pool_xhat(float xf, float mu, float is) {
+#pragma clang fp contract(off)
+  return (xf - mu) * is;
+}
+
+__device__ __forceinline__ float bn_pool_dx(float w, float g, float db,
+                                            float xhat, float ds) {
+#pragma clang fp contract(off)
+  const float t = g - db;
+  return w * fmaf(-xhat, ds, t);
+}
+
+__device__ __forceinline__ unsigned char bn_mask_byte(const ushort8& o) {
+  unsigned int m = 0;
+#pragma unroll
+  for (int j = 0; j < 8; j++)
+    m |= (bf16_to_f32(o[j]) > 0.f ? 1u : 0u) << j;
+  return (unsigned char)m;
+}
+
 struct BnGeom {
   long long M;
   int C, CG, blocks, stat_blocks;
 };
 
 BnGeom bn_geom_of(const torch::Tensor& x);
+
+void bn_check_mask(const torch::Tensor& mask, const torch::Tensor& x,
+                   const BnGeom& g);
 
 void bn_launch_fwd_stats(const torch::Tensor& x, const BnGeom& g,
                          const torch::Tensor& weight,
diff --git a/kubeshare_amd/ops/hip/bn_join.hip b/kubeshare_amd/ops/hip/bn_join.hip
--- /dev/null
+++ b/kubeshare_amd/ops/hip/bn_join.hip
@@ -0,0 +1,396 @@
+#include <hip/hip_runtime.h>
+#include <torch/extension.h>
+#include <ATen/cuda/CUDAContext.h>
+
+#include <vector>
+
+#include "bn_common.h"
+
+#define KS_BN_JOIN_U 2
+#define KS_BN_JOIN_U1 1
+#define KS_BN_JOIN_UA 1
+
+template <bool MASK>
+__global__ void bn_join_apply_kernel(const ushort8* __restrict__ x,
+                                     const ushort8* __restrict__ xd,
+                                     ushort8* __restrict__ y,
+                                     unsigned char* __restrict__ mask,
+                                     const float* __restrict__ scale,
+                                     const float* __restrict__ biasf,
+                                     const float* __restrict__ scale_d,
+                                     const float* __restrict__ biasf_d,
+                                     long long M, int CG) {
+  const int tid = threadIdx.x;
+  const int cg = tid % CG;
+  const int roff = tid / CG;
+  const int rows_per_blk = KS_BN_BLOCK / CG;
+  const bool active = roff < rows_per_blk;
+  const long long stride = (long long)gridDim.x * rows_per_blk;
+  float8 s, b, sd, bd;
+#pragma unroll
+  for (int j = 0; j < 8; j++) {
+    s[j] = scale[cg * 8 + j];
+    b[j] = biasf[cg * 8 + j];
+    sd[j] = scale_d[cg * 8 + j];
+    bd[j] = biasf_d[cg * 8 + j];
+  }
+  auto one = [&](const ushort8& v, const ushort8& vd) {
+    ushort8 o;
+#pragma unroll
+    for (int j = 0; j < 8; j++) {
+      const float id = bf16_to_f32(
+          f32_to_bf16(bn_affine(bf16_to_f32(vd[j]), sd[j], bd[j])));
+      float f = bn_affine(bf16_to_f32(v[j]), s[j], b[j]);
+      f += id;
+      o[j] = bn_relu_bf16(f);
+    }
+    return o;
+  };
+  long long row = active ? (long long)blockIdx.x * rows_per_blk + roff : M;
+  for (; row + (KS_BN_UNROLL - 1) * stride < M;
+       row += KS_BN_UNROLL * stride) {
+    ushort8 v[KS_BN_UNROLL], vd[KS_BN_UNROLL];
+    long long k[KS_BN_UNROLL];
+#pragma unroll
+    for (int u = 0; u < KS_BN_UNROLL; u++) {
+      k[u] = (row + u * stride) * CG + cg;
+      v[u] = x[k[u]];
+      vd[u] = xd[k[u]];
+    }
+#pragma unroll
+    for (int u = 0; u < KS_BN_UNROLL; u++) {
+      const ushort8 o = one(v[u], vd[u]);
+      y[k[u]] = o;
+      if (MASK) mask[k[u]] = bn_mask_byte(o);
+    }
+  }
+  for (; row < M; row += stride) {
+    const long long k = row * CG + cg;
+    const ushort8 o = one(x[k], xd[k]);
+    y[k] = o;
+    if (MASK) mask[k] = bn_mask_byte(o);
+  }
+}
+
+template <bool WITH_DY2, bool MASK>
+__global__ void bn_join_bwd_stats_kernel(
+    const ushort8* __restrict__ x, const ushort8* __restrict__ xd,
+    const ushort8* __restrict__ y, const unsigned char* __restrict__ mask,
+    const ushort8* __restrict__ dy, const ushort8* __restrict__ dy2,
+    ushort8* __restrict__ dym_out, const float* __restrict__ mean,
+    const float* __restrict__ invstd, const float* __restrict__ mean_d,
+    const float* __restrict__ invstd_d, float* __restrict__ part,
+    float* __restrict__ part_d, long long M, int CG) {
+  __shared__ float s_red[KS_BN_BLOCK * 8];
+  const int tid = threadIdx.x;
+  const int cg = tid % CG;
+  const int roff = tid / CG;
+  const int rows_per_blk = KS_BN_BLOCK / CG;
+  const bool active = roff < rows_per_blk;
+  const long long stride = (long long)gridDim.x * rows_per_blk;
+  float8 mu, is, mud, isd;
+#pragma unroll
+  for (int j = 0; j < 8; j++) {
+    mu[j] = mean[cg * 8 + j];
+    is[j] = invstd[cg * 8 + j];
+    mud[j] = mean_d[cg * 8 + j];
+    isd[j] = invstd_d[cg * 8 + j];
+  }
+  float8 adb = {0, 0, 0, 0, 0, 0, 0, 0};
+  float8 ads = {0, 0, 0, 0, 0, 0, 0, 0};
+  float8 adsd = {0, 0, 0, 0, 0, 0, 0, 0};
+  constexpr int U = WITH_DY2 ? KS_BN_JOIN_U : KS_BN_JOIN_U1;
+  static_assert(KS_BN_UNROLL % U == 0, "sub-batches must tile a group");
+  long long row = active ? (long long)blockIdx.x * rows_per_blk + roff : M;
+  for (; row + (KS_BN_UNROLL - 1) * stride < M;
+       row += KS_BN_UNROLL * stride) {
+#pragma unroll 1
+    for (int h = 0; h < KS_BN_UNROLL; h += U) {
+      ushort8 xv[U], xdv[U], yv[U], gv[U], g2[U];
+      unsigned char mv[U];
+      long long k[U];
+#pragma unroll
+      for (int u = 0; u < U; u++) {
+        k[u] = (row + (h + u) * stride) * CG + cg;
+        xv[u] = x[k[u]];
+        xdv[u] = xd[k[u]];
+        if (MASK) mv[u] = mask[k[u]]; else yv[u] = y[k[u]];
+        gv[u] = dy[k[u]];
+        if (WITH_DY2) g2[u] = dy2[k[u]];
+      }
+#pragma unroll
+      for (int u = 0; u < U; u++) {
+        ushort8 dm;
+#pragma unroll
+        for (int j = 0; j < 8; j++) {
+          const float gin = WITH_DY2 ? bn_join_grad(gv[u][j], g2[u][j])
+                                     : bf16_to_f32(gv[u][j]);
+          const bool on = MASK ? ((mv[u] >> j) & 1) != 0
+                               : bf16_to_f32(yv[u][j]) > 0.f;
+          const float g = on ? gin : 0.f;
+          adb[j] += g;
+          ads[j] = bn_acc_dscale<true>(
+              ads[j], g, bn_pool_xhat(bf16_to_f32(xv[u][j]), mu[j], is[j]),
+              j);
+          adsd[j] = bn_acc_dscale<true>(
+              adsd[j], g,
+              bn_pool_xhat(bf16_to_f32(xdv[u][j]), mud[j], isd[j]), j);
+          dm[j] = f32_to_bf16(g);
+        }
+        dym_out[k[u]] = dm;
+      }
+    }
+  }
+  for (; row < M; row += stride) {
+    const long long k = row * CG + cg;
+    const ushort8 xv = x[k], xdv = xd[k], gv = dy[k];
+    ushort8 yv, g2;
+    unsigned char mv;
+    if (MASK) mv = mask[k]; else yv = y[k];
+    if (WITH_DY2) g2 = dy2[k];
+    ushort8 dm;
+#pragma unroll
+    for (int j = 0; j < 8; j++) {
+      const float gin =
+          WITH_DY2 ? bn_join_grad(gv[j], g2[j]) : bf16_to_f32(gv[j]);
+      const bool on = MASK ? ((mv >> j) & 1) != 0 : bf16_to_f32(yv[j]) > 0.f;
+      const float g = on ? gin : 0.f;
+      adb[j] += g;
+      ads[j] = bn_acc_dscale<false>(
+          ads[j], g, bn_pool_xhat(bf16_to_f32(xv[j]), mu[j], is[j]), j);
+      adsd[j] = bn_acc_dscale<false>(
+          adsd[j], g, bn_pool_xhat(bf16_to_f32(xdv[j]), mud[j], isd[j]), j);
+      dm[j] = f32_to_bf16(g);
+    }
+    dym_out[k] = dm;
+  }
+
+  const int C = CG * 8;
+  float* const outs[3] = {part + (long long)blockIdx.x * C,
+                          part + (long long)(gridDim.x + blockIdx.x) * C,
+                          part_d + (long long)blockIdx.x * C};
+#pragma unroll
+  for (int q = 0; q < 3; q++) {
+    const float8& a = q == 0 ? adb : q == 1 ? ads : adsd;
+    if (q) __syncthreads();
+#pragma unroll
+    for (int j = 0; j < 8; j++) s_red[tid * 8 + j] = a[j];
+    __syncthreads();
+    if (tid < CG) {
+      float8 t = {0, 0, 0, 0, 0, 0, 0, 0};
+      for (int r = 0; r < rows_per_blk; r++)
+#pragma unroll
+        for (int j = 0; j < 8; j++) t[j] += s_red[(r * CG + tid) * 8 + j];
+#pragma unroll
+      for (int j = 0; j < 8; j++) outs[q][tid * 8 + j] = t[j];
+    }
+  }
+}
+
+__global__ void bn_join_bwd_apply_kernel(
+    const ushort8* __restrict__ x, const ushort8* __restrict__ xd,
+    const ushort8* __restrict__ dym, ushort8* __restrict__ dx,
+    ushort8* __restrict__ dxd, const float* __restrict__ mean,
+    const float* __restrict__ invstd, const float* __restrict__ weight,
+    const float* __restrict__ mean_d, const float* __restrict__ invstd_d,
+    const float* __restrict__ weight_d, const float* __restrict__ dbias,
+    const float* __restrict__ dscale, const float* __restrict__ dscale_d,
+    long long M, int CG) {
+  const int tid = threadIdx.x;
+  const int cg = tid % CG;
+  const int roff = tid / CG;
+  const int rows_per_blk = KS_BN_BLOCK / CG;
+  const bool active = roff < rows_per_blk;
+  const long long stride = (long long)gridDim.x * rows_per_blk;
+  const float invM = 1.f / (float)M;
+  float8 mu, is, w, ds, mud, isd, wd, dsd, db;
+#pragma unroll
+  for (int j = 0; j < 8; j++) {
+    const int c = cg * 8 + j;
+    mu[j] = mean[c];
+    is[j] = invstd[c];
+    w[j] = weight[c] * is[j];
+    ds[j] = dscale[c] * invM;
+    mud[j] = mean_d[c];
+    isd[j] = invstd_d[c];
+    wd[j] = weight_d[c] * isd[j];
+    dsd[j] = dscale_d[c] * invM;
+    db[j] = dbias[c] * invM;
+  }
+  constexpr int U = KS_BN_JOIN_UA;
+  long long row = active ? (long long)blockIdx.x * rows_per_blk + roff : M;
+  for (; row + (U - 1) * stride < M; row += U * stride) {
+    ushort8 xv[U], xdv[U], gv[U];
+    long long k[U];
+#pragma unroll
+    for (int u = 0; u < U; u++) {
+      k[u] = (row + u * stride) * CG + cg;
+      xv[u] = x[k[u]];
+      xdv[u] = xd[k[u]];
+      gv[u] = dym[k[u]];
+    }
+#pragma unroll
+    for (int u = 0; u < U; u++) {
+      ushort8 o, od;
+#pragma unroll
+      for (int j = 0; j < 8; j++) {
+        const float g = bf16_to_f32(gv[u][j]);
+        o[j] = f32_to_bf16(bn_pool_dx(
+            w[j], g, db[j],
+            bn_pool_xhat(bf16_to_f32(xv[u][j]), mu[j], is[j]), ds[j]));
+        od[j] = f32_to_bf16(bn_pool_dx(
+            wd[j], g, db[j],
+            bn_pool_xhat(bf16_to_f32(xdv[u][j]), mud[j], isd[j]), dsd[j]));
+      }
+      dx[k[u]] = o;
+      dxd[k[u]] = od;
+    }
+  }
+  for (; row < M; row += stride) {
+    const long long k = row * CG + cg;
+    const ushort8 xv = x[k], xdv = xd[k], gv = dym[k];
+    ushort8 o, od;
+#pragma unroll
+    for (int j = 0; j < 8; j++) {
+      const float g = bf16_to_f32(gv[j]);
+      o[j] = f32_to_bf16(bn_pool_dx(
+          w[j], g, db[j], bn_pool_xhat(bf16_to_f32(xv[j]), mu[j], is[j]),
+          ds[j]));
+      od[j] = f32_to_bf16(bn_pool_dx(
+          wd[j], g, db[j],
+          bn_pool_xhat(bf16_to_f32(xdv[j]), mud[j], isd[j]), dsd[j]));
+    }
+    dx[k] = o;
+    dxd[k] = od;
+  }
+}
+
+namespace {
+
+void check_pair(const torch::Tensor& x, const torch::Tensor& x_d,
+                const char* what) {
+  TORCH_CHECK(x_d.is_cuda() && x_d.sizes() == x.sizes() &&
+                  x_d.scalar_type() == at::kBFloat16 &&
+                  x_d.is_contiguous(at::MemoryFormat::ChannelsLast),
+              what, ": x_d must be channels-last bf16 of x's shape");
+}
+
+const ushort8* cptr(const torch::Tensor& t) {
+  return reinterpret_cast<const ushort8*>(t.data_ptr());
+}
+
+ushort8* mptr(torch::Tensor& t) {
+  return reinterpret_cast<ushort8*>(t.data_ptr());
+}
+
+}
+
+std::vector<torch::Tensor> bn_join_fwd_train(
+    torch::Tensor x, torch::Tensor weight, torch::Tensor bias,
+    torch::Tensor running_mean, torch::Tensor running_var, double momentum,
+    double eps, torch::Tensor x_d, torch::Tensor weight_d,
+    torch::Tensor bias_d, torch::Tensor running_mean_d,
+    torch::Tensor running_var_d, double momentum_d, double eps_d,
+    bool want_mask, bool legacy_reduce) {
+  BnGeom g = bn_geom_of(x);
+  check_pair(x, x_d, "bn_join_fwd_train");
+  auto stream = at::cuda::getCurrentCUDAStream();
+  auto f32 = x.options().dtype(at::kFloat);
+  auto y = at::empty_like(x);
+  auto mean = at::empty({g.C}, f32), invstd = at::empty({g.C}, f32);
+  auto mean_d = at::empty({g.C}, f32), invstd_d = at::empty({g.C}, f32);
+  auto scale = at::empty({g.C}, f32), biasf = at::empty({g.C}, f32);
+  auto scale_d = at::empty({g.C}, f32), biasf_d = at::empty({g.C}, f32);
+  auto fptr = [](torch::Tensor& t) {
+    return t.defined() ? t.data_ptr<float>() : nullptr;
+  };
+  bn_launch_fwd_stats(x_d, g, weight_d, bias_d, fptr(running_mean_d),
+                      fptr(running_var_d), mean_d, invstd_d, scale_d, biasf_d,
+                      momentum_d, eps_d, legacy_reduce, stream.stream());
+  bn_launch_fwd_stats(x, g, weight, bias, fptr(running_mean),
+                      fptr(running_var), mean, invstd, scale, biasf, momentum,
+                      eps, legacy_reduce, stream.stream());
+  torch::Tensor mask;
+  if (want_mask)
+    mask = at::empty({x.size(0), x.size(2), x.size(3), (long long)g.CG},
+                     x.options().dtype(at::kByte));
+  auto launch = [&](auto kern) {
+    hipLaunchKernelGGL(kern, dim3(g.blocks), dim3(KS_BN_BLOCK), 0,
+                       stream.stream(), cptr(x), cptr(x_d), mptr(y),
+                       want_mask ? mask.data_ptr<unsigned char>() : nullptr,
+                       scale.data_ptr<float>(), biasf.data_ptr<float>(),
+                       scale_d.data_ptr<float>(), biasf_d.data_ptr<float>(),
+                       g.M, g.CG);
+  };
+  want_mask ? launch(bn_join_apply_kernel<true>)
+            : launch(bn_join_apply_kernel<false>);
+  if (want_mask) return {y, mean, invstd, mean_d, invstd_d, mask};
+  return {y, mean, invstd, mean_d, invstd_d};
+}
+
+std::vector<torch::Tensor> bn_join_bwd(
+    torch::Tensor x, torch::Tensor x_d, torch::Tensor y_or_mask,
+    torch::Tensor dy, c10::optional<torch::Tensor> dy2, torch::Tensor weight,
+    torch::Tensor weight_d, torch::Tensor mean, torch::Tensor invstd,
+    torch::Tensor mean_d, torch::Tensor invstd_d, bool use_mask,
+    bool legacy_reduce) {
+  BnGeom g = bn_geom_of(x);
+  check_pair(x, x_d, "bn_join_bwd");
+  TORCH_CHECK(dy.sizes() == x.sizes() && dy.scalar_type() == at::kBFloat16,
+              "bn_join_bwd: dy must be bf16 of x's shape");
+  if (use_mask)
+    bn_check_mask(y_or_mask, x, g);
+  else
+    check_pair(x, y_or_mask, "bn_join_bwd (y)");
+  bool fold_dy2 = false;
+  if (dy2.has_value() && dy2->defined()) {
+    TORCH_CHECK(dy2->sizes() == x.sizes(),
+                "bn_join_bwd: dy2 must have x's shape");
+    fold_dy2 = dy2->is_cuda() && dy2->scalar_type() == at::kBFloat16 &&
+               dy2->is_contiguous(at::MemoryFormat::ChannelsLast) &&
+               dy.is_contiguous(at::MemoryFormat::ChannelsLast);
+    if (!fold_dy2) dy = (dy + *dy2).to(at::kBFloat16);
+  }
+  if (!dy.is_contiguous(at::MemoryFormat::ChannelsLast))
+    dy = dy.contiguous(at::MemoryFormat::ChannelsLast);
+  auto stream = at::cuda::getCurrentCUDAStream();
+  auto f32 = x.options().dtype(at::kFloat);
+  auto part = at::empty({(long long)3 * g.stat_blocks * g.C}, f32);
+  float* part_p = part.data_ptr<float>();
+  float* part_d_p = part_p + (long long)2 * g.stat_blocks * g.C;
+  auto red = at::empty({g.C * 3}, f32);
+  float* dbias_p = red.data_ptr<float>();
+  float* dscale_p = dbias_p + g.C;
+  float* dscale_d_p = dscale_p + g.C;
+  auto dym = at::empty_like(x);
+  auto dx = at::empty_like(x);
+  auto dx_d = at::empty_like(x);
+  auto launch_stats = [&](auto kern) {
+    hipLaunchKernelGGL(
+        kern, dim3(g.stat_blocks), dim3(KS_BN_BLOCK), 0, stream.stream(),
+        cptr(x), cptr(x_d), use_mask ? nullptr : cptr(y_or_mask),
+        use_mask ? y_or_mask.data_ptr<unsigned char>() : nullptr, cptr(dy),
+        fold_dy2 ? cptr(*dy2) : nullptr, mptr(dym), mean.data_ptr<float>(),
+        invstd.data_ptr<float>(), mean_d.data_ptr<float>(),
+        invstd_d.data_ptr<float>(), part_p, part_d_p, g.M, g.CG);
+  };
+  if (use_mask)
+    fold_dy2 ? launch_stats(bn_join_bwd_stats_kernel<true, true>)
+             : launch_stats(bn_join_bwd_stats_kernel<false, true>);
+  else
+    fold_dy2 ? launch_stats(bn_join_bwd_stats_kernel<true, false>)
+             : launch_stats(bn_join_bwd_stats_kernel<false, false>);
+  bn_launch_bwd_reduce(part_p, g.stat_blocks, g.C, dbias_p, dscale_p,
+                       legacy_reduce, stream.stream());
+  bn_launch_reduce_one(part_d_p, g.stat_blocks, g.C, dscale_d_p,
+                       stream.stream());
+  hipLaunchKernelGGL(bn_join_bwd_apply_kernel, dim3(g.blocks),
+                     dim3(KS_BN_BLOCK), 0, stream.stream(), cptr(x),
+                     cptr(x_d), cptr(dym), mptr(dx), mptr(dx_d),
+                     mean.data_ptr<float>(), invstd.data_ptr<float>(),
+                     weight.data_ptr<float>(), mean_d.data_ptr<float>(),
+                     invstd_d.data_ptr<float>(), weight_d.data_ptr<float>(),
+                     dbias_p, dscale_p, dscale_d_p, g.M, g.CG);
+  return {dx, dx_d, red.narrow(0, g.C, g.C), red.narrow(0, 0, g.C),
+          red.narrow(0, 2 * g.C, g.C)};
+}
diff --git a/kubeshare_amd/ops/hip/bn_pool.hip b/kubeshare_amd/ops/hip/bn_pool.hip
--- a/kubeshare_amd/ops/hip/bn_pool.hip
+++ b/kubeshare_amd/ops/hip/bn_pool.hip
@@ -155,17 +155,6 @@
   return f32_to_bf16(f > 0.f ? f : 0.f) != 0;
 }
 
-__device__ __forceinline__ float bn_pool_xhat(float xf, float mu, float is) {
-#pragma clang fp contract(off)
-  return (xf - mu) * is;
-}
-
-__device__ __forceinline__ float bn_pool_dx(float w, float g, float db,
-                                            float xhat, float ds) {
-#pragma clang fp contract(off)
-  const float t = g - db;
-  return w * fmaf(-xhat, ds, t);
-}
 
 __device__ __forceinline__ float bn_pool_fold_scale(float w, float is) {
   return w * is;
diff --git a/kubeshare_amd/ops/hip/bn_relu.hip b/kubeshare_amd/ops/hip/bn_relu.hip
--- a/kubeshare_amd/ops/hip/bn_relu.hip
+++ b/kubeshare_amd/ops/hip/bn_relu.hip
@@ -227,10 +227,11 @@
   bn_finalize_channel(f, c, sum[c], sumsq[c]);
 }
 
-template <bool WITH_RES, bool RELU = true>
+template <bool WITH_RES, bool RELU = true, bool MASK = false>
 __global__ void bn_apply_relu_kernel(const ushort8* __restrict__ x,
                                      const ushort8* __restrict__ res,
                                      ushort8* __restrict__ y,
+                                     unsigned char* __restrict__ mask,
                                      const float* __restrict__ scale,
                                      const float* __restrict__ biasf,
                                      long long M, int CG) {
@@ -266,6 +267,7 @@
         o[u][j] = RELU ? bn_relu_bf16(f) : f32_to_bf16(f);
       }
       y[k[u]] = o[u];
+      if (MASK) mask[k[u]] = bn_mask_byte(o[u]);
     }
   }
   for (; row < M; row += stride) {
@@ -281,17 +283,14 @@
       o[j] = RELU ? bn_relu_bf16(f) : f32_to_bf16(f);
     }
     y[k] = o;
-  }
-}
-
-__device__ __forceinline__ float bn_join_grad(unsigned short a,
-                                              unsigned short b) {
-  return bf16_to_f32(f32_to_bf16(bf16_to_f32(a) + bf16_to_f32(b)));
-}
-
-template <bool WRITE_DYM, bool WITH_DY2 = false>
+    if (MASK) mask[k] = bn_mask_byte(o);
+  }
+}
+
+template <bool WRITE_DYM, bool WITH_DY2 = false, bool MASK = false>
 __global__ void bn_bwd_stats_kernel(const ushort8* __restrict__ x,
                                     const ushort8* __restrict__ y,
+                                    const unsigned char* __restrict__ mask,
                                     const ushort8* __restrict__ dy,
                                     const ushort8* __restrict__ dy2,
                                     ushort8* __restrict__ dym_out,
@@ -314,7 +313,7 @@
   }
   float8 adb = {0, 0, 0, 0, 0, 0, 0, 0};
   float8 ads = {0, 0, 0, 0, 0, 0, 0, 0};
-  constexpr int U = WITH_DY2 ? KS_BN_UNROLL_DY2 : KS_BN_UNROLL;
+  constexpr int U = (WITH_DY2 || MASK) ? KS_BN_UNROLL_DY2 : KS_BN_UNROLL;
   static_assert(KS_BN_UNROLL % U == 0, "sub-batches must tile a group");
   long long row = active ? (long long)blockIdx.x * rows_per_blk + roff : M;
   for (; row + (KS_BN_UNROLL - 1) * stride < M;
@@ -323,12 +322,13 @@
     for (int h = 0; h < KS_BN_UNROLL; h += U) {
       ushort8 xv[U], yv[U], gv[U];
       ushort8 g2[U];
+      unsigned char mv[U];
       long long k[U];
 #pragma unroll
       for (int u = 0; u < U; u++) {
         k[u] = (row + (h + u) * stride) * CG + cg;
         xv[u] = x[k[u]];
-        yv[u] = y[k[u]];
+        if (MASK) mv[u] = mask[k[u]]; else yv[u] = y[k[u]];
         gv[u] = dy[k[u]];
         if (WITH_DY2) g2[u] = dy2[k[u]];
       }
@@ -339,7 +339,9 @@
         for (int j = 0; j < 8; j++) {
           float gin = WITH_DY2 ? bn_join_grad(gv[u][j], g2[u][j])
                                : bf16_to_f32(gv[u][j]);
-          float g = bf16_to_f32(yv[u][j]) > 0.f ? gin : 0.f;
+          const bool on = MASK ? ((mv[u] >> j) & 1) != 0
+                               : bf16_to_f32(yv[u][j]) > 0.f;
+          float g = on ? gin : 0.f;
           float xhat = (bf16_to_f32(xv[u][j]) - mu[j]) * is[j];
           adb[j] += g;
           ads[j] = bn_acc_dscale<true>(ads[j], g, xhat, j);
@@ -351,14 +353,18 @@
   }
   for (; row < M; row += stride) {
     const long long k = row * CG + cg;
-    ushort8 xv = x[k], yv = y[k], gv = dy[k];
+    ushort8 xv = x[k], gv = dy[k];
+    ushort8 yv;
+    unsigned char mv;
+    if (MASK) mv = mask[k]; else yv = y[k];
     ushort8 g2;
     if (WITH_DY2) g2 = dy2[k];
     ushort8 dm;
 #pragma unroll
     for (int j = 0; j < 8; j++) {
       float gin = WITH_DY2 ? bn_join_grad(gv[j], g2[j]) : bf16_to_f32(gv[j]);
-      float g = bf16_to_f32(yv[j]) > 0.f ? gin : 0.f;
+      const bool on = MASK ? ((mv >> j) & 1) != 0 : bf16_to_f32(yv[j]) > 0.f;
+      float g = on ? gin : 0.f;
       float xhat = (bf16_to_f32(xv[j]) - mu[j]) * is[j];
       adb[j] += g;
       ads[j] = bn_acc_dscale<false>(ads[j], g, xhat, j);
@@ -707,6 +713,15 @@
   float s = weight[c] * rsqrtf(rvar[c] + eps);
   scale_out[c] = s;
   bias_out[c] = bias[c] - rmean[c] * s;
+}
+
+void bn_check_mask(const torch::Tensor& mask, const torch::Tensor& x,
+                   const BnGeom& g) {
+  TORCH_CHECK(mask.is_cuda() && mask.scalar_type() == at::kByte &&
+                  mask.is_contiguous() && mask.dim() == 4 &&
+                  mask.size(0) == x.size(0) && mask.size(1) == x.size(2) &&
+                  mask.size(2) == x.size(3) && mask.size(3) == g.CG,
+              "ReLU mask must be a contiguous uint8 (N, H, W, C/8) tensor");
 }
 
 BnGeom bn_geom_of(const torch::Tensor& x) {
@@ -810,11 +825,18 @@
     torch::Tensor x, torch::Tensor weight, torch::Tensor bias,
     torch::Tensor running_mean, torch::Tensor running_var, double momentum,
     double eps, c10::optional<torch::Tensor> res, bool relu,
-    bool legacy_reduce) {
+    bool legacy_reduce, bool want_mask) {
   BnGeom g = bn_geom_of(x);
+  TORCH_CHECK(!want_mask || (res.has_value() && relu),
+              "bn_relu_fwd_train: the ReLU mask is for residual BNs with "
+              "ReLU");
   auto stream = at::cuda::getCurrentCUDAStream();
   auto f32 = x.options().dtype(at::kFloat);
   auto y = at::empty_like(x);
+  torch::Tensor mask;
+  if (want_mask)
+    mask = at::empty({x.size(0), x.size(2), x.size(3), (long long)g.CG},
+                     x.options().dtype(at::kByte));
   auto save_mean = at::empty({g.C}, f32);
   auto save_invstd = at::empty({g.C}, f32);
   auto scale = at::empty({g.C}, f32);
@@ -834,15 +856,19 @@
                            ? reinterpret_cast<const ushort8*>(res->data_ptr())
                            : nullptr,
                        reinterpret_cast<ushort8*>(y.data_ptr()),
+                       want_mask ? mask.data_ptr<unsigned char>() : nullptr,
                        scale.data_ptr<float>(), biasf.data_ptr<float>(), g.M,
                        g.CG);
   };
-  if (res.has_value())
+  if (want_mask)
+    launch_apply(bn_apply_relu_kernel<true, true, true>);
+  else if (res.has_value())
     relu ? launch_apply(bn_apply_relu_kernel<true, true>)
          : launch_apply(bn_apply_relu_kernel<true, false>);
   else
     relu ? launch_apply(bn_apply_relu_kernel<false, true>)
          : launch_apply(bn_apply_relu_kernel<false, false>);
+  if (want_mask) return {y, save_mean, save_invstd, mask};
   return {y, save_mean, save_invstd};
 }
 
@@ -866,8 +892,8 @@
                            ? reinterpret_cast<const ushort8*>(res->data_ptr())
                            : nullptr,
                        reinterpret_cast<ushort8*>(y.data_ptr()),
-                       scale.data_ptr<float>(), biasf.data_ptr<float>(), g.M,
-                       g.CG);
+                       (unsigned char*)nullptr, scale.data_ptr<float>(),
+                       biasf.data_ptr<float>(), g.M, g.CG);
   };
   if (res.has_value())
     relu ? launch_apply(bn_apply_relu_kernel<true, true>)
@@ -878,19 +904,26 @@
   return y;
 }
 
-std::vector<torch::Tensor> bn_relu_bwd(torch::Tensor x, torch::Tensor y,
-                                       torch::Tensor dy, torch::Tensor weight,
-                                       torch::Tensor bias, torch::Tensor mean,
-                                       torch::Tensor invstd, bool need_dres,
-                                       bool relu,
-                                       c10::optional<torch::Tensor> dy2,
-                                       bool legacy_reduce) {
+std::vector<torch::Tensor> bn_relu_bwd(
+    torch::Tensor x, c10::optional<torch::Tensor> y, torch::Tensor dy,
+    torch::Tensor weight, torch::Tensor bias, torch::Tensor mean,
+    torch::Tensor invstd, bool need_dres, bool relu,
+    c10::optional<torch::Tensor> dy2, bool legacy_reduce,
+    c10::optional<torch::Tensor> mask) {
   TORCH_CHECK(relu || !need_dres,
               "bn_relu_bwd: residual path requires the ReLU variant");
   BnGeom g = bn_geom_of(x);
-  TORCH_CHECK(dy.sizes() == x.sizes() && y.sizes() == x.sizes() &&
-                  dy.scalar_type() == at::kBFloat16,
+  TORCH_CHECK(dy.sizes() == x.sizes() && dy.scalar_type() == at::kBFloat16,
               "bn_relu_bwd: dy must be bf16 of x's shape");
+  const bool use_mask = need_dres && mask.has_value() && mask->defined();
+  if (use_mask) {
+    bn_check_mask(*mask, x, g);
+  } else if (need_dres) {
+    TORCH_CHECK(y.has_value() && y->defined() && y->sizes() == x.sizes() &&
+                    y->scalar_type() == at::kBFloat16 &&
+                    y->is_contiguous(at::MemoryFormat::ChannelsLast),
+                "bn_relu_bwd: y must be channels-last bf16 of x's shape");
+  }
   bool fold_dy2 = false;
   if (dy2.has_value() && dy2->defined()) {
     TORCH_CHECK(dy2->sizes() == x.sizes(),
@@ -922,7 +955,10 @@
       hipLaunchKernelGGL(kern, dim3(g.stat_blocks), dim3(KS_BN_BLOCK), 0,
                          stream.stream(),
                          reinterpret_cast<const ushort8*>(x.data_ptr()),
-                         reinterpret_cast<const ushort8*>(y.data_ptr()),
+                         use_mask ? nullptr
+                                  : reinterpret_cast<const ushort8*>(
+                                        y->data_ptr()),
+                         use_mask ? mask->data_ptr<unsigned char>() : nullptr,
                          reinterpret_cast<const ushort8*>(dy.data_ptr()),
                          fold_dy2 ? reinterpret_cast<const ushort8*>(
                                         dy2->data_ptr())
@@ -931,8 +967,12 @@
                          mean.data_ptr<float>(), invstd.data_ptr<float>(),
                          part.data_ptr<float>(), g.M, g.CG);
     };
-    fold_dy2 ? launch_rstats(bn_bwd_stats_kernel<true, true>)
-             : launch_rstats(bn_bwd_stats_kernel<true, false>);
+    if (use_mask)
+      fold_dy2 ? launch_rstats(bn_bwd_stats_kernel<true, true, true>)
+               : launch_rstats(bn_bwd_stats_kernel<true, false, true>);
+    else
+      fold_dy2 ? launch_rstats(bn_bwd_stats_kernel<true, true>)
+               : launch_rstats(bn_bwd_stats_kernel<true, false>);
     launch_reduce();
     hipLaunchKernelGGL(bn_bwd_apply_dym_kernel, dim3(g.blocks),
                        dim3(KS_BN_BLOCK), 0, stream.stream(),
diff --git a/kubeshare_amd/ops/hip/ks_ops.hip b/kubeshare_amd/ops/hip/ks_ops.hip
--- a/kubeshare_amd/ops/hip/ks_ops.hip
+++ b/kubeshare_amd/ops/hip/ks_ops.hip
@@ -260,18 +260,31 @@
     torch::Tensor x, torch::Tensor weight, torch::Tensor bias,
     torch::Tensor running_mean, torch::Tensor running_var, double momentum,
     double eps, c10::optional<torch::Tensor> res, bool relu,
-    bool legacy_reduce);
+    bool legacy_reduce, bool want_mask);
 torch::Tensor bn_relu_fwd_eval(torch::Tensor x, torch::Tensor weight,
                                torch::Tensor bias, torch::Tensor rmean,
                                torch::Tensor rvar, double eps,
                                c10::optional<torch::Tensor> res, bool relu);
-std::vector<torch::Tensor> bn_relu_bwd(torch::Tensor x, torch::Tensor y,
-                                       torch::Tensor dy, torch::Tensor weight,
-                                       torch::Tensor bias, torch::Tensor mean,
-                                       torch::Tensor invstd, bool need_dres,
-                                       bool relu,
-                                       c10::optional<torch::Tensor> dy2,
-                                       bool legacy_reduce);
+std::vector<torch::Tensor> bn_relu_bwd(
+    torch::Tensor x, c10::optional<torch::Tensor> y, torch::Tensor dy,
+    torch::Tensor weight, torch::Tensor bias, torch::Tensor mean,
+    torch::Tensor invstd, bool need_dres, bool relu,
+    c10::optional<torch::Tensor> dy2, bool legacy_reduce,
+    c10::optional<torch::Tensor> mask);
+
+std::vector<torch::Tensor> bn_join_fwd_train(
+    torch::Tensor x, torch::Tensor weight, torch::Tensor bias,
+    torch::Tensor running_mean, torch::Tensor running_var, double momentum,
+    double eps, torch::Tensor x_d, torch::Tensor weight_d,
+    torch::Tensor bias_d, torch::Tensor running_mean_d,
+    torch::Tensor running_var_d, double momentum_d, double eps_d,
+    bool want_mask, bool legacy_reduce);
+std::vector<torch::Tensor> bn_join_bwd(
+    torch::Tensor x, torch::Tensor x_d, torch::Tensor y_or_mask,
+    torch::Tensor dy, c10::optional<torch::Tensor> dy2, torch::Tensor weight,
+    torch::Tensor weight_d, torch::Tensor mean, torch::Tensor invstd,
+    torch::Tensor mean_d, torch::Tensor invstd_d, bool use_mask,
+    bool legacy_reduce);
 
 std::vector<c10::optional<torch::Tensor>> cast_f32_to_bf16_multi(
     std::vector<c10::optional<torch::Tensor>> src);
@@ -322,12 +335,33 @@
   m.def("bn_relu_fwd_train", &bn_relu_fwd_train, py::arg("x"),
         py::arg("weight"), py::arg("bias"), py::arg("running_mean"),
         py::arg("running_var"), py::arg("momentum"), py::arg("eps"),
-        py::arg("res"), py::arg("relu"), py::arg("legacy_reduce") = false);
+        py::arg("res"), py::arg("relu"), py::arg("legacy_reduce") = false,
+        py::arg("want_mask") = false,
+        "{y, mean, invstd} and, with want_mask (res and relu only), the "
+        "uint8 (N, H, W, C/8) ReLU mask");
   m.def("bn_relu_fwd_eval", &bn_relu_fwd_eval);
   m.def("bn_relu_bwd", &bn_relu_bwd, py::arg("x"), py::arg("y"),
         py::arg("dy"), py::arg("weight"), py::arg("bias"), py::arg("mean"),
         py::arg("invstd"), py::arg("need_dres"), py::arg("relu"),
-        py::arg("dy2") = py::none(), py::arg("legacy_reduce") = false);
+        py::arg("dy2") = py::none(), py::arg("legacy_reduce") = false,
+        py::arg("mask") = py::none(),
+        "{dx, dscale, dbias[, dres]}; with mask (residual BNs) y may be "
+        "None");
+  m.def("bn_join_fwd_train", &bn_join_fwd_train, py::arg("x"),
+        py::arg("weight"), py::arg("bias"), py::arg("running_mean"),
+        py::arg("running_var"), py::arg("momentum"), py::arg("eps"),
+        py::arg("x_d"), py::arg("weight_d"), py::arg("bias_d"),
+        py::arg("running_mean_d"), py::arg("running_var_d"),
+        py::arg("momentum_d"), py::arg("eps_d"), py::arg("want_mask"),
+        py::arg("legacy_reduce") = false,
+        "relu(bn(x) + bn_d(x_d)): {y, mean, invstd, mean_d, invstd_d} and, "
+        "with want_mask, the uint8 (N, H, W, C/8) ReLU mask");
+  m.def("bn_join_bwd", &bn_join_bwd, py::arg("x"), py::arg("x_d"),
+        py::arg("y_or_mask"), py::arg("dy"), py::arg("dy2"),
+        py::arg("weight"), py::arg("weight_d"), py::arg("mean"),
+        py::arg("invstd"), py::arg("mean_d"), py::arg("invstd_d"),
+        py::arg("use_mask"), py::arg("legacy_reduce") = false,
+        "{dx, dx_d, dscale, dbias, dscale_d}; dbias serves both BNs");
   m.def("cast_f32_to_bf16_multi", &cast_f32_to_bf16_multi,
         "f32 -> bf16 (torch rounding) of every tensor of a list in as few "
         "launches as the kernel-argument limit allows; None stays None");
```

Measured after the change: 9458 images/s, median of 6. +3.4%, better.
